# cisco/openh264

Measured on AMD Instinct MI355X. Metric: 1080p frames/sec/GPU at QP=24 CBP; encoder_binary_comparison SHA1 pass, higher is better.
Workload: dtype u8

## Files before the change

integration/welship_isvc.cpp:

```cpp
#include <dlfcn.h>
#include <stdio.h>
#include <stdlib.h>
#include <string.h>
#include <string>
#include <vector>
#include "codec_api.h"
#include "../include/welship.h"

namespace {

struct Api {
  void* so = nullptr;
  int (*Create) (WelsHipEncoder**) = nullptr;
  void (*Destroy) (WelsHipEncoder*) = nullptr;
  int (*GetDefaultParams) (WelsHipEncoder*, WelsHipEncParam*) = nullptr;
  int (*InitializeExt) (WelsHipEncoder*, const WelsHipEncParam*) = nullptr;
  int (*Uninitialize) (WelsHipEncoder*) = nullptr;
  int (*EncodeFrame) (WelsHipEncoder*, const WelsHipSourcePicture*, WelsHipFrameBSInfo*) = nullptr;
  int (*ForceIntraFrame) (WelsHipEncoder*, int) = nullptr;
  int (*GetReconFrame) (WelsHipEncoder*, uint8_t*, size_t) = nullptr;
  int (*SetOption) (WelsHipEncoder*, int, void*) = nullptr;
  int (*EncodeParameterSets) (WelsHipEncoder*, WelsHipFrameBSInfo*) = nullptr;
  int (*GetOption) (WelsHipEncoder*, int, void*) = nullptr;
  const char* (*GetLastError) (void) = nullptr;
  int (*GetFrameQuality) (WelsHipEncoder*, WelsHipFrameQuality*) = nullptr;
  bool load() {
    if (so) return true;
    const char* path = getenv ("WELSHIP_LIB");
    so = dlopen (path && *path ? path : "libwelship.so", RTLD_NOW | RTLD_LOCAL);
    if (!so) { fprintf (stderr, "welship_isvc: cannot open the engine library (%s): %s\n", path ? path : "libwelship.so", dlerror()); return false; }
#define SYM(field, name) field = reinterpret_cast<decltype (field)> (dlsym (so, name)); if (!field) { fprintf (stderr, "welship_isvc: missing symbol %s\n", name); return false; }
    SYM (Create, "WelsHipCreateEncoder") SYM (Destroy, "WelsHipDestroyEncoder") SYM (GetDefaultParams, "WelsHipGetDefaultParams")
    SYM (InitializeExt, "WelsHipInitializeExt") SYM (Uninitialize, "WelsHipUninitialize") SYM (EncodeFrame, "WelsHipEncodeFrame")
    SYM (ForceIntraFrame, "WelsHipForceIntraFrame") SYM (GetLastError, "WelsHipGetLastError") SYM (GetReconFrame, "WelsHipGetReconFrame")
    SYM (SetOption, "WelsHipSetOption") SYM (GetOption, "WelsHipGetOption") SYM (EncodeParameterSets, "WelsHipEncodeParameterSets")
    SYM (GetFrameQuality, "WelsHipGetFrameQuality")
#undef SYM
    return true;
  }
} g_api;

class CWelsHipEncoder : public ISVCEncoder {
 public:
  CWelsHipEncoder() { if (g_api.load()) g_api.Create (&m_p); }
  virtual ~CWelsHipEncoder() { if (m_p) g_api.Destroy (m_p); }
  bool Ok() const { return m_p != NULL; }

  virtual int EXTAPI Initialize (const SEncParamBase* b) {
    if (!b) return cmInitParaError;
    SEncParamExt e;
    GetDefaultParams (&e);
    e.iUsageType = b->iUsageType; e.iPicWidth = b->iPicWidth; e.iPicHeight = b->iPicHeight;
    e.iTargetBitrate = b->iTargetBitrate; e.iRCMode = b->iRCMode; e.fMaxFrameRate = b->fMaxFrameRate;
    e.sSpatialLayers[0].iVideoWidth = b->iPicWidth; e.sSpatialLayers[0].iVideoHeight = b->iPicHeight;
    e.sSpatialLayers[0].fFrameRate = b->fMaxFrameRate; e.sSpatialLayers[0].iSpatialBitrate = b->iTargetBitrate;
    return InitializeExt (&e);
  }
  virtual int EXTAPI InitializeExt (const SEncParamExt* p) {
    if (!p || !m_p) return cmInitParaError;
    WelsHipEncParam q;
    g_api.GetDefaultParams (m_p, &q);
    q.iUsageType = p->iUsageType; q.iPicWidth = p->iPicWidth; q.iPicHeight = p->iPicHeight;
    q.iTargetBitrate = p->sSpatialLayers[0].iSpatialBitrate > 0 ? p->sSpatialLayers[0].iSpatialBitrate : p->iTargetBitrate;
    q.iRCMode = p->iRCMode; q.fMaxFrameRate = p->fMaxFrameRate;
    q.iTemporalLayerNum = p->iTemporalLayerNum; q.iSpatialLayerNum = p->iSpatialLayerNum;
    q.iComplexityMode = p->iComplexityMode; q.uiIntraPeriod = p->uiIntraPeriod;
    q.eSpsPpsIdStrategy = p->eSpsPpsIdStrategy; q.iEntropyCodingModeFlag = p->iEntropyCodingModeFlag;
    q.iLoopFilterDisableIdc = p->iLoopFilterDisableIdc; q.iLoopFilterAlphaC0Offset = p->iLoopFilterAlphaC0Offset;
    q.iLoopFilterBetaOffset = p->iLoopFilterBetaOffset; q.bEnableFrameCroppingFlag = p->bEnableFrameCroppingFlag;
    const SSpatialLayerConfig& l = p->sSpatialLayers[0];
    q.iDLayerQp = l.iDLayerQp;
    q.uiSliceMode = l.sSliceArgument.uiSliceMode; q.uiSliceNum = l.sSliceArgument.uiSliceNum;
    for (int k = 0; k < MAX_SLICES_NUM_TMP && k < 35; ++k) q.uiSliceMbNum[k] = l.sSliceArgument.uiSliceMbNum[k];
    q.bEnableAdaptiveQuant = p->bEnableAdaptiveQuant; q.bEnableBackgroundDetection = p->bEnableBackgroundDetection;
    q.bEnableSceneChangeDetect = p->bEnableSceneChangeDetect; q.bEnableLongTermReference = p->bEnableLongTermReference;
    q.bEnableDenoise = p->bEnableDenoise; q.bEnableFrameSkip = p->bEnableFrameSkip;
    q.iMultipleThreadIdc = p->iMultipleThreadIdc;
    q.bPsnrY = p->bPsnrY; q.bPsnrU = p->bPsnrU; q.bPsnrV = p->bPsnrV;
    m_param_planes = (p->bPsnrY ? 1 : 0) | (p->bPsnrU ? 2 : 0) | (p->bPsnrV ? 4 : 0);
    const int rc = g_api.InitializeExt (m_p, &q);
    if (rc) fprintf (stderr, "welship_isvc: InitializeExt: %s\n", g_api.GetLastError());
    m_w = p->iPicWidth; m_h = p->iPicHeight; m_frames = 0;
    return rc;
  }
  virtual int EXTAPI GetDefaultParams (SEncParamExt* p) {
    if (!p) return cmInitParaError;
    memset (p, 0, sizeof (*p));
    WelsHipEncParam q;
    if (m_p) g_api.GetDefaultParams (m_p, &q); else memset (&q, 0, sizeof (q));
    p->iUsageType = (EUsageType)q.iUsageType; p->iRCMode = (RC_MODES)q.iRCMode; p->fMaxFrameRate = q.fMaxFrameRate;
    p->iTemporalLayerNum = q.iTemporalLayerNum; p->iSpatialLayerNum = q.iSpatialLayerNum;
    p->iComplexityMode = (ECOMPLEXITY_MODE)q.iComplexityMode; p->uiIntraPeriod = q.uiIntraPeriod;
    p->eSpsPpsIdStrategy = (EParameterSetStrategy)q.eSpsPpsIdStrategy; p->iEntropyCodingModeFlag = q.iEntropyCodingModeFlag;
    p->iLoopFilterDisableIdc = q.iLoopFilterDisableIdc; p->bEnableFrameCroppingFlag = q.bEnableFrameCroppingFlag != 0;
    p->iMultipleThreadIdc = 1; p->iNumRefFrame = 1; p->iMaxQp = 51; p->iMinQp = 0;
    p->sSpatialLayers[0].iDLayerQp = q.iDLayerQp; p->sSpatialLayers[0].uiProfileIdc = PRO_BASELINE;
    p->sSpatialLayers[0].sSliceArgument.uiSliceMode = SM_SINGLE_SLICE; p->sSpatialLayers[0].sSliceArgument.uiSliceNum = 1;
    return cmResultSuccess;
  }
  virtual int EXTAPI Uninitialize() { return m_p ? g_api.Uninitialize (m_p) : cmInitParaError; }
  virtual int EXTAPI EncodeFrame (const SSourcePicture* s, SFrameBSInfo* o) {
    if (!s || !o || !m_p) return cmInitParaError;
    WelsHipSourcePicture sp;
    memset (&sp, 0, sizeof (sp));
    sp.iColorFormat = s->iColorFormat;
    for (int k = 0; k < 4; ++k) { sp.iStride[k] = s->iStride[k]; sp.pData[k] = s->pData[k]; }
    sp.iPicWidth = s->iPicWidth; sp.iPicHeight = s->iPicHeight; sp.uiTimeStamp = s->uiTimeStamp;
    const int pic_planes = (s->bPsnrY ? 1 : 0) | (s->bPsnrU ? 2 : 0) | (s->bPsnrV ? 4 : 0);
    int planes = m_param_planes | pic_planes;
    if (g_api.SetOption (m_p, WELSHIP_OPTION_PSNR_PLANES, &planes)) return cmInitParaError;
    WelsHipFrameBSInfo b;
    const int rc = g_api.EncodeFrame (m_p, &sp, &b);
    if (rc) { fprintf (stderr, "welship_isvc: EncodeFrame: %s\n", g_api.GetLastError()); return rc; }
    memset (o, 0, sizeof (*o));
    o->iLayerNum = b.iLayerNum; o->eFrameType = (EVideoFrameType)b.eFrameType;
    o->iFrameSizeInBytes = b.iFrameSizeInBytes; o->uiTimeStamp = b.uiTimeStamp;
    for (int i = 0; i < b.iLayerNum; ++i) {
      o->sLayerInfo[i].uiLayerType = b.sLayerInfo[i].uiLayerType; o->sLayerInfo[i].eFrameType = (EVideoFrameType)b.sLayerInfo[i].eFrameType;
      o->sLayerInfo[i].uiTemporalId = b.sLayerInfo[i].uiTemporalId; o->sLayerInfo[i].uiSpatialId = b.sLayerInfo[i].uiSpatialId;
      o->sLayerInfo[i].uiQualityId = b.sLayerInfo[i].uiQualityId; o->sLayerInfo[i].iSubSeqId = b.sLayerInfo[i].iSubSeqId;
      o->sLayerInfo[i].iNalCount = b.sLayerInfo[i].iNalCount; o->sLayerInfo[i].pNalLengthInByte = b.sLayerInfo[i].pNalLengthInByte;
      o->sLayerInfo[i].pBsBuf = b.sLayerInfo[i].pBsBuf;
    }
    if (pic_planes) {
      WelsHipFrameQuality fq;
      if (g_api.GetFrameQuality (m_p, &fq)) return cmUnknownReason;
      for (int i = 0; i < b.iLayerNum; ++i)
        if (b.sLayerInfo[i].uiLayerType == WELSHIP_VIDEO_CODING_LAYER)
          for (int k = 0; k < 3; ++k) o->sLayerInfo[i].rPsnr[k] = ((pic_planes >> k) & 1) ? fq.rPsnr[k] : 0.0f;
    }
    if (!m_dump.empty() && b.eFrameType != WelsHipFrameTypeSkip) {
      std::vector<uint8_t> rec ((size_t)m_w * m_h * 3 / 2);
      if (g_api.GetReconFrame (m_p, rec.data(), rec.size()) == 0) {
        FILE* f = fopen (m_dump.c_str(), m_frames == 0 ? "wb" : "ab");
        if (f) { fwrite (rec.data(), 1, rec.size(), f); fclose (f); }
      }
    }
    ++m_frames;
    return cmResultSuccess;
  }
  virtual int EXTAPI EncodeParameterSets (SFrameBSInfo* o) {
    if (!o || !m_p) return cmInitParaError;
    WelsHipFrameBSInfo b;
    const int rc = g_api.EncodeParameterSets (m_p, &b);
    if (rc) return rc;
    memset (o, 0, sizeof (*o));
    o->iLayerNum = 1; o->eFrameType = videoFrameTypeInvalid; o->iFrameSizeInBytes = b.iFrameSizeInBytes;
    o->sLayerInfo[0].uiLayerType = NON_VIDEO_CODING_LAYER; o->sLayerInfo[0].eFrameType = videoFrameTypeInvalid;
    o->sLayerInfo[0].iNalCount = b.sLayerInfo[0].iNalCount; o->sLayerInfo[0].pNalLengthInByte = b.sLayerInfo[0].pNalLengthInByte;
    o->sLayerInfo[0].pBsBuf = b.sLayerInfo[0].pBsBuf;
    return cmResultSuccess;
  }
  virtual int EXTAPI ForceIntraFrame (bool bIdr, int = -1) { return m_p ? g_api.ForceIntraFrame (m_p, bIdr ? 1 : 0) : cmInitParaError; }
  virtual int EXTAPI SetOption (ENCODER_OPTION id, void* pOption) {
    if (id == ENCODER_OPTION_DUMP_FILE && pOption) {
      const SDumpLayer* d = static_cast<const SDumpLayer*> (pOption);
      if (d->iLayer != 0 || !d->pFileName) return cmInitParaError;
      m_dump = d->pFileName;
      return cmResultSuccess;
    }
    if (id == ENCODER_OPTION_TRACE_LEVEL || id == ENCODER_OPTION_TRACE_CALLBACK || id == ENCODER_OPTION_TRACE_CALLBACK_CONTEXT) return cmResultSuccess;
    return m_p ? g_api.SetOption (m_p, (int)id, pOption) : cmInitExpected;
  }
  virtual int EXTAPI GetOption (ENCODER_OPTION id, void* pOption) { return m_p ? g_api.GetOption (m_p, (int)id, pOption) : cmInitExpected; }

 private:
  WelsHipEncoder* m_p = NULL;
  std::string m_dump;
  int m_w = 0, m_h = 0, m_frames = 0;
  int m_param_planes = 0;
};

}

extern "C" int WelsCreateSVCEncoder (ISVCEncoder** ppEncoder) {
  if (!ppEncoder) return 1;
  CWelsHipEncoder* e = new CWelsHipEncoder();
  if (!e->Ok()) { delete e; *ppEncoder = NULL; return 1; }
  *ppEncoder = e;
  return 0;
}
extern "C" void WelsDestroySVCEncoder (ISVCEncoder* pEncoder) { delete static_cast<CWelsHipEncoder*> (pEncoder); }
```

openh264_amd/csrc/common/wh_types.h:

```cpp
#pragma once
#include <stdint.h>

#ifdef __cplusplus
extern "C" {
#endif

enum {
  WH_MB_I4x4   = 0,
  WH_MB_I16x16 = 1,
  WH_MB_P16x16 = 2,
  WH_MB_P16x8  = 3,
  WH_MB_P8x16  = 4,
  WH_MB_P8x8   = 5,
  WH_MB_PSKIP  = 6,
  WH_MB_NONE   = 255
};
#define WH_IS_INTRA(t) ((t) <= WH_MB_I16x16)
#define WH_IS_INTER(t) ((t) >= WH_MB_P16x16 && (t) <= WH_MB_PSKIP)
#define WH_REFTYPE_BACKGROUND 64

enum { WH_SLICE_P = 0, WH_SLICE_I = 2 };

typedef struct WhMbRecord {
  uint8_t  mb_type;
// ... 58 lines not shown
  const uint32_t* fme_start;
  const uint16_t* fme_loc;
  int32_t fme_list_size;
  int32_t scd_on;
  uint32_t* chain;
  uint32_t* fme_cost_down;
  uint32_t* chain_mb;
} WhSccJob;

#define WH_GOM_MAX 160

typedef struct WhGomRc {
  int32_t n_gom_mb;
  int32_t end_mb;
  int32_t target_bits;
  int32_t min_qp, max_qp;
  int32_t slice_qp;
  int32_t p_slice;
  int32_t pad;
  int32_t gom_sad[WH_GOM_MAX];
  int32_t calc_qp;
  int32_t frame_bits;
  int32_t gom_bits;
  int32_t gom_target;
  int32_t index;
  int32_t skip_run, last_qp;
  int32_t pad2;
} WhGomRc;

typedef struct WhPicJob {
  const uint8_t* src[3];
  uint8_t*       rec[3];
  const uint8_t* ref[3];
  WhMbRecord*    records;
  WhMbState*     mbs;
  const WhMbState* ref_mbs;
  int32_t        qp;
  int32_t        slice_type;
  const WhMbCtl* mb_ctl;
  int32_t        ref_is_p;
  int32_t        want_bits;
  const uint8_t* prev_src_y;
  uint32_t*      db_flags;
  uint32_t       db_gen;
  int32_t        dyn_first;
  uint32_t*      scene_count;
  int32_t*       sad_cost0;
  const int32_t* vaa_sad8x8;
  const int8_t*  bgd_flags;
  int32_t        mvc_shift;
  int32_t        mb_begin;
  int32_t        mb_end;
  int32_t        dyn_slice;
  uint8_t*       compact;
  uint32_t*      compact_off;
  const int16_t* il_hint;
  const WhSccJob* scc;
  const uint32_t* scc_order;
  const int32_t* scc_chain_prev;
  WhGomRc* gom_rc;
  int32_t*       sad_cost0_out;
  int32_t        dyn_redo;
  uint32_t       sse_planes;
  uint8_t*       rec_tiles[2];
  const uint8_t* ref_tiles[2];
  uint8_t*       rec_blk;
  uint64_t*      sse;
} WhPicJob;

#define WH_SRC_MB_BYTES 384
#define WH_SRC_Y_OFF(mb_w, mbx, mby, row, x) ((size_t) ((mby) * (mb_w) + (mbx)) * WH_SRC_MB_BYTES + (size_t) ((row) * 16 + (x)))
#define WH_SRC_C_OFF(mb_w, mbx, mby, pl, row, x) ((size_t) ((mby) * (mb_w) + (mbx)) * WH_SRC_MB_BYTES + (size_t) (256 + (pl) * 64 + (row) * 8 + (x)))
#define WH_TILE_BYTES 128
#define WH_TILE_Y_OFF(stride_y, x, y) ((((size_t) (((y) + 32) >> 3) * (size_t) ((stride_y) >> 4) + (size_t) (((x) + 32) >> 4)) << 7) + (size_t) ((((y) + 32) & 7) << 4))
#define WH_TILE_C_OFF(stride_c, x, y) ((((size_t) (((y) + 16) >> 3) * (size_t) ((stride_c) >> 3) + (size_t) (((x) + 16) >> 3)) << 7) + (size_t) ((((y) + 16) & 7) << 4))

#define WH_MAX_SLICES 36
#define WH_SEQ_SCC 1
#define WH_SEQ_SERIAL 2
#define WH_SEQ_CHAIN 4
#define WH_SEQ_PLAIN 32
#define WH_SEQ_NO_CTRL 64
#define WH_SEQ_DB_WHOLE 16
#define WH_SEQ_RANGED 8
#define WH_DB_WHOLE_TABLE(P) ((P).db_bands + 3 * (size_t)(P).db_num_bands + 1)
#define WH_DB_BAND_ROWS 24

typedef struct WhSeqParams {
  int32_t mb_w, mb_h;
  int32_t src_stride_y, src_stride_c;
  int32_t rec_stride_y, rec_stride_c;
  int32_t complexity;
  int32_t chroma_qp_offset;
  int32_t num_slices;
  int32_t slice_first_mb[WH_MAX_SLICES + 1];
  int32_t deblock_idc;
  int32_t alpha_offset, beta_offset;
  int32_t mv_range;
  int32_t flags;
  int32_t blk8_w, blk8_h;
  unsigned long long* prof;
  const uint32_t* mb_order;
  int32_t db_num_bands, db_max_mbs;
  const int32_t* db_bands;
  int32_t db_max_rows;
} WhSeqParams;

#ifdef __cplusplus
}
#endif
```

openh264_amd/csrc/hip/hip_backend.hip:

```cpp
#include <hip/hip_runtime.h>
#include <stdio.h>
#include <stdlib.h>
#include <string>
#include <vector>
#include <algorithm>
#include <map>
#include <unordered_map>
#include <atomic>
#include "../host/backend.h"
#include "../kernels/frame_kernels.h"
#include <mutex>
#include "../kernels/deblock_mb.h"
#include "../kernels/inter_mb.h"
#include "../kernels/expand_pic.h"
#include "../kernels/tile_pic.h"
#include "../kernels/vaa_pic.h"
#include "../kernels/bgd_pic.h"
#include "../kernels/scene_pic.h"
#include "../kernels/quality_pic.h"
#include "../common/compact.h"

namespace {

#define WH_NUM_QUEUES 32
#define WH_ERR_WORDS 4
#define WH_SEAM_SPIN_LIMIT (1u << 22)
#define WH_SPIN_LIMIT (1u << 23)

__device__ __forceinline__ bool wh_wait_done (const uint32_t* done, int idx, uint32_t* err) {
  if (idx < 0) return true;
  uint32_t spins = 0;
  while (!((__hip_atomic_load (&done[idx >> 5], __ATOMIC_RELAXED, __HIP_MEMORY_SCOPE_WORKGROUP) >> (idx & 31)) & 1u)) {
    __builtin_amdgcn_s_sleep (4);
    if (++spins > WH_SPIN_LIMIT) {
      if ((threadIdx.x & 63) == 0 && atomicAdd (err, 1u) == 0) { err[1] = blockIdx.x; err[2] = blockIdx.y; err[3] = (uint32_t)idx; }
      return false;
    }
  }
  return true;
}

__device__ __forceinline__ WhMbLds& wh_prof_holder (WhInterLds& S) { return S.m; }
__device__ __forceinline__ WhMbLds& wh_prof_holder (WhMbLds& S) { return S; }
__device__ __forceinline__ WhMbLds& wh_prof_holder (WhDbLds& S) { return * (WhMbLds*)&S; }
#if defined(WH_PROF)
template <class T> __device__ __forceinline__ uint32_t* wh_prof_lds (T& S) { return wh_prof_holder (S).prof; }
#define WH_PROF_ON 1
#else
template <class T> __device__ __forceinline__ uint32_t* wh_prof_lds (T& S) { return nullptr; }
#define WH_PROF_ON 0
#endif

__device__ __forceinline__ void wh_copy_job (WhPicJob* dst, const WhPicJob* src) {
  for (unsigned i = threadIdx.x; i < sizeof (WhPicJob) / 4; i += blockDim.x) ((uint32_t*)dst)[i] = ((const uint32_t*)src)[i];
}

#define WH_DEFINE_MB_KERNEL(NAME, LDS_T, BODY, MAX_THREADS, WHOLE_PICTURE, PROF, GOM)                                             \
__global__ __launch_bounds__ (MAX_THREADS) void NAME (WhSeqParams P, const WhPicJob* jobs, uint32_t* err) {             \
  extern __shared__ __align__ (16) uint8_t smem[];                                                                      \
  const int nw = (int)blockDim.x >> 6, lane = (int)threadIdx.x & 63;                                                    \
  const int wave = __builtin_amdgcn_readfirstlane ((int)threadIdx.x >> 6);      \
  LDS_T& S = ((LDS_T*)smem)[wave];                                                                                      \
  uint32_t* sched = (uint32_t*) (smem + (size_t)nw * sizeof (LDS_T));           \
  const int num_mb = P.mb_w * P.mb_h;                                                                                   \
  const int first = WHOLE_PICTURE ? 0 : P.slice_first_mb[blockIdx.x];                                                   \
  const int n = WHOLE_PICTURE ? num_mb : P.slice_first_mb[blockIdx.x + 1] - first;                                      \
  const uint32_t* order0 = P.mb_order + (WHOLE_PICTURE ? num_mb : first);                                               \
  for (int i = (int)threadIdx.x; i < 1 + ((n + 31) >> 5); i += (int)blockDim.x) sched[i] = 0;                          \
  if (WH_PROF_ON && PROF && P.prof && lane < 32) wh_prof_lds (S)[lane] = 0;                                                           \
  __shared__ WhPicJob Jl;                           \
  wh_copy_job (&Jl, &jobs[blockIdx.y]);                                                                                 \
  __syncthreads();                                                                                                      \
  WH_PROF_DECL (P);                                                                                                     \
  const WhPicJob& J = Jl;                                                                                               \
   \
   \
  const uint32_t* order = (GOM && J.gom_rc) ? (const uint32_t*)J.scc_order + first : order0;                                     \
  for (int guard = 0; guard <= n; ++guard) {                         \
    int t = 0;                                                                                                          \
    if (lane == 0) t = (int)atomicAdd (&sched[0], 1u);                                                                  \
    t = __builtin_amdgcn_readfirstlane (t);                                                                             \
    if (t >= n) break;                                                                                                  \
    const int xy = order[t];                                                                                            \
    if (PROF) WH_PROF_MARK (P, wh_prof_holder (S), 11);                                       \
    if (J.mb_end > 0) {                              \
      if (xy < J.mb_begin) { if (lane == 0) atomicOr (&sched[1 + ((xy - first) >> 5)], 1u << ((xy - first) & 31)); continue; } \
      if (xy >= J.mb_end) continue;                                                                                     \
    }                                                                                                                   \
    int dep_a, dep_b;                                                                                                   \
    wh_mb_deps (P.mb_w, xy, first, &dep_a, &dep_b);                                                                     \
    if (!wh_wait_done (sched + 1, dep_a < 0 ? -1 : dep_a - first, err)) break;        \
    if (!wh_wait_done (sched + 1, dep_b < 0 ? -1 : dep_b - first, err)) break;                                          \
    if (GOM && J.gom_rc) { const int dep_c = ((const WH_G int32_t*)J.scc_chain_prev)[xy]; if (!wh_wait_done (sched + 1, dep_c < first ? -1 : dep_c - first, err)) break; } \
    __builtin_amdgcn_fence (__ATOMIC_ACQUIRE, "workgroup");                                                             \
    if (PROF) WH_PROF_MARK (P, wh_prof_holder (S), 12);                                             \
    BODY (S, P, J, xy % P.mb_w, xy / P.mb_w);                                                                           \
    if (GOM && J.gom_rc) wh_gom_close_if_last (P, J, xy);     \
    if (PROF) WH_PROF_MARK (P, wh_prof_holder (S), 14);                \
// ... 248 lines not shown
#define WH_XCLAIM()                                                                                                            \
  {                                                                                                                            \
    int tt = 0;                                                                                                                \
    if (lane == 0) tt = (int)__hip_atomic_fetch_add (&sc[0], 1u, __ATOMIC_RELAXED, __HIP_MEMORY_SCOPE_AGENT);                  \
    tt = __builtin_amdgcn_readfirstlane (tt);                                                                                  \
    xy = -1;                                                                                                                   \
    if (tt < n) {                                                                                                              \
      xy = (int)order[tt];                                                                                                     \
      mby = P.mb_w > 1 ? (int)__umulhi ((uint32_t)xy, w_rcp) : xy; mbx = xy - mby * P.mb_w;                                    \
      WhPicJob Jf;                                                                                                             \
      Jf.src[0] = J.src[0]; Jf.prev_src_y = J.prev_src_y; Jf.ref_mbs = J.ref_mbs; Jf.ref_is_p = J.ref_is_p;                    \
      Jf.ref_tiles[0] = J.ref_tiles[0]; Jf.ref_tiles[1] = J.ref_tiles[1];                                                      \
      if (HOSTIN) { Jf.vaa_sad8x8 = J.vaa_sad8x8; Jf.sad_cost0 = J.sad_cost0; }                                                \
      const int guess_ = slot_mv;                                                                                              \
      wh_inter_cold_fetch<VAR> (S, G, lane, P, Jf, mbx, mby);                                                                  \
      wh_win_speculate (P, Jf, X.spec, mbx, mby, guess_); X.spec_valid = 1;                                                    \
    }                                                                                                                          \
  }
  WH_XCLAIM()
  while (xy >= 0) {
    const int dep_a = (mbx > 0 && xy - 1 >= first) ? xy - 1 : -1;
    int dep_b;
    { const int tr = mbx < P.mb_w - 1 ? xy - P.mb_w + 1 : xy - P.mb_w; dep_b = tr >= first ? tr : -1; }
    if (!wh_wait_done_x (sc + 1, dep_a < 0 ? -1 : dep_a - first, err)) break;
    if (!wh_wait_done_x (sc + 1, dep_b < 0 ? -1 : dep_b - first, err)) break;
    __builtin_amdgcn_fence (__ATOMIC_ACQUIRE, "workgroup");
    WV_ASYNC_WAIT();
    wh_inter_mb_body_t<false, VAR, true> (S, G, P, J, mbx, mby, X);
    asm volatile ("s_waitcnt vmcnt(0)" ::: "memory");
    if (lane == 0) __hip_atomic_fetch_or (&sc[1 + ((xy - first) >> 5)], 1u << ((xy - first) & 31), __ATOMIC_RELAXED, __HIP_MEMORY_SCOPE_SYSTEM);
    WH_XCLAIM()
  }
#undef WH_XCLAIM
#if WH_PROF_ON
  if (P.prof && lane < 32) atomicAdd (&P.prof[((blockIdx.x * 7u) & 63u) * 32u + lane], (unsigned long long)S.m.prof[lane]);
#endif
}

__global__ __launch_bounds__ (1024) void k_md_assign (uint32_t* slice_cost, uint16_t* groups, int n, int n_groups, int slots) {
  __shared__ uint32_t key[4096];
  __shared__ uint16_t val[4096];
  int m = 1;
  while (m < n) m <<= 1;
  for (int i = (int)threadIdx.x; i < m; i += (int)blockDim.x) { key[i] = i < n ? slice_cost[i] : 0u; val[i] = (uint16_t) (i < n ? i : 0xffff); }
  __syncthreads();
  for (int i = (int)threadIdx.x; i < n; i += (int)blockDim.x) slice_cost[i] = 0;
  for (int k = 2; k <= m; k <<= 1)
    for (int j = k >> 1; j > 0; j >>= 1) {
      for (int i = (int)threadIdx.x; i < m; i += (int)blockDim.x) {
        const int l = i ^ j;
        if (l > i) {
          const bool up = (i & k) == 0;
          const uint32_t a = key[i], b = key[l];
          const bool sw = up ? (a < b || (a == b && val[i] == 0xffff && val[l] != 0xffff)) : (a > b);
          if (sw) { key[i] = b; key[l] = a; const uint16_t t = val[i]; val[i] = val[l]; val[l] = t; }
        }
      }
      __syncthreads();
    }
  for (int g = (int)threadIdx.x; g < n_groups * slots; g += (int)blockDim.x) groups[g] = 0xffff;
  __shared__ int wtot[17];
  int carry = 0;
  const int lane = (int)threadIdx.x & 63, wave = (int)threadIdx.x >> 6, nwv = (int)blockDim.x >> 6;
  for (int base = 0; base < m; base += (int)blockDim.x) {
    const int i = base + (int)threadIdx.x;
    const bool valid = i < m && val[i] != 0xffff;
    const unsigned long long b = __ballot (valid);
    const int before = __builtin_popcountll (b & ((1ull << lane) - 1ull));
    __syncthreads();
    if (lane == 0) wtot[wave] = __builtin_popcountll (b);
    __syncthreads();
    if (threadIdx.x == 0) { int acc = 0; for (int w2 = 0; w2 < nwv; ++w2) { const int t = wtot[w2]; wtot[w2] = acc; acc += t; } wtot[16] = acc; }
    __syncthreads();
    if (valid) {
      const int p = carry + wtot[wave] + before;
      const int r = p / n_groups, c = p % n_groups;
      const int g = (r & 1) ? n_groups - 1 - c : c;
      if (r < slots) groups[g * slots + r] = val[i];
    }
    carry += wtot[16];
  }
}

__global__ __launch_bounds__ (1024) void k_deblock_slices (WhSeqParams P, const WhPicJob* jobs, uint32_t* err) {
  extern __shared__ __align__ (16) uint8_t smem[];
  const int nw = (int)blockDim.x >> 6, lane = (int)threadIdx.x & 63;
  const int wave = __builtin_amdgcn_readfirstlane ((int)threadIdx.x >> 6);
  WhDbLds& S = ((WhDbLds*)smem)[wave];
  WhDbXchg E;
  E.top = (uint32_t*) (smem + (size_t)nw * sizeof (WhDbLds));
  E.left = E.top + (size_t)P.mb_w * 24;
  E.first_row = 0;
  uint32_t* sched = E.left + (size_t)P.mb_h * 32;
  const int w = P.mb_w, num_mb = P.mb_w * P.mb_h;
  const int nb = P.db_num_bands;
  const int first = P.db_bands[blockIdx.x], last = P.db_bands[blockIdx.x + 1], n = last - first;
  const bool cross = P.deblock_idc == 0;
  const int sfirst = cross ? 0 : P.db_bands[nb + 1 + blockIdx.x], slast = cross ? num_mb : P.db_bands[2 * nb + 1 + blockIdx.x];
  const uint32_t* order = (P.flags & WH_SEQ_DB_WHOLE) ? P.mb_order + num_mb : P.mb_order + 2 * num_mb + first;
  for (int i = (int)threadIdx.x; i < 1 + ((n + 31) >> 5); i += (int)blockDim.x) sched[i] = 0;
  __shared__ WhPicJob Jl;
  wh_copy_job (&Jl, &jobs[blockIdx.y]);
  __syncthreads();
  const WhPicJob& J = Jl;
  uint32_t* flags = J.db_flags;
  const uint32_t gen = J.db_gen;
  __shared__ WhDbStage stage[16];
  WhDbStage& G = stage[wave];
#if WH_PROF_ON
  if (P.prof && lane < 32) S.prof[lane] = 0;
#endif
  WH_PROF_DECL (P);
  for (int guard = 0; guard <= n; ++guard) {
    int t = 0;
    if (lane == 0) t = (int)atomicAdd (&sched[0], 1u);
    t = __builtin_amdgcn_readfirstlane (t);
    if (t >= n) break;
    const int xy = order[t];
    WH_PROF_MARK (P, S, 0);
    wh_deblock_cold_fetch (G, lane, P, J, xy % w, xy / w);
    WH_PROF_MARK (P, S, 1);
    int dep_a, dep_b;
    wh_mb_deps (w, xy, 0, &dep_a, &dep_b);
    bool remote = false, ok = true;
    for (int k = 0; k < 2 && ok; ++k) {
      const int dep = k == 0 ? dep_a : dep_b;
      if (dep < 0) continue;
      if (dep >= first) ok = wh_wait_done (sched + 1, dep - first, err);
      else if (dep >= sfirst) {
        uint32_t spins = 0;
        while (__hip_atomic_load (&flags[dep], __ATOMIC_RELAXED, __HIP_MEMORY_SCOPE_SYSTEM) != gen) {
          __builtin_amdgcn_s_sleep (8);
          if (++spins > WH_SEAM_SPIN_LIMIT) { if (lane == 0 && atomicAdd (err, 1u) == 0) { err[1] = blockIdx.x; err[2] = blockIdx.y; err[3] = 0x80000000u | (uint32_t)dep; } ok = false; break; }
        }
        remote = true;
      }
    }
    if (!ok) break;
    __builtin_amdgcn_fence (__ATOMIC_ACQUIRE, "workgroup");
    WH_PROF_MARK (P, S, remote ? 3 : 2);
    WV_ASYNC_WAIT();
    WH_PROF_MARK (P, S, 4);
    const bool publish = xy + w + 1 >= last && last < slast;
    const bool drain = wh_deblock_mb_body (S, G, E, first, last, P, J, xy % w, xy / w, 0, 0, 0, publish);
    WH_PROF_MARK (P, S, 11);
    if (publish) {
      asm volatile ("s_waitcnt vmcnt(0)" ::: "memory");
      if (lane == 0) __hip_atomic_store (&flags[xy], gen, __ATOMIC_RELAXED, __HIP_MEMORY_SCOPE_SYSTEM);
    } else if (drain) {
      __builtin_amdgcn_fence (__ATOMIC_RELEASE, "workgroup");
    }
    WV_SYNC();
    if (lane == 0) atomicOr (&sched[1 + ((xy - first) >> 5)], 1u << ((xy - first) & 31));
    WH_PROF_MARK (P, S, 9);
  }
  WH_PROF_MARK (P, S, 10);
#if WH_PROF_ON
  if (P.prof && lane < 32) atomicAdd (&P.prof[2048u + ((blockIdx.x + blockIdx.y * 7u) & 63u) * 32u + lane], (unsigned long long)S.prof[lane]);
#endif
}


#ifndef WH_DB_ITEMS_IN_LDS
#define WH_DB_ITEMS_IN_LDS 1
#endif
#define WH_DB_ITEMS_LDS_MAX_MB 9216
__global__ __launch_bounds__ (1024) void k_deblock_pairs (WhSeqParams P, const WhPicJob* jobs, uint32_t* err) {
  extern __shared__ __align__ (16) uint8_t smem[];
  const int nw = (int)blockDim.x >> 6, lane = (int)threadIdx.x & 63;
  const int wave = __builtin_amdgcn_readfirstlane ((int)threadIdx.x >> 6);
  WhDbLds* S2 = (WhDbLds*)smem + 2 * wave;
  WhDbLds& S = S2[0];
  WhDbXchg E;
  E.top = (uint32_t*) (smem + (size_t)nw * 2 * sizeof (WhDbLds));
  E.left = E.top + (size_t)P.mb_w * 24;
  E.first_row = 0;
  uint32_t* sched = E.left + (size_t)P.mb_h * 32;
  const int w = P.mb_w, num_mb = P.mb_w * P.mb_h;
  const uint32_t* items_g = P.mb_order + 3 * (size_t)num_mb;
  const int n = (int)items_g[0];
  for (int i = (int)threadIdx.x; i < 1 + ((num_mb + 31) >> 5); i += (int)blockDim.x) sched[i] = 0;
#if WH_DB_ITEMS_IN_LDS
  uint32_t* items_l = sched + 1 + ((num_mb + 31) >> 5);
  const bool items_in_lds = num_mb <= WH_DB_ITEMS_LDS_MAX_MB;
  if (items_in_lds) for (int i = (int)threadIdx.x; i <= n; i += (int)blockDim.x) items_l[i] = items_g[i];
#else
  const bool items_in_lds = false; uint32_t* items_l = nullptr;
#endif
  __shared__ WhPicJob Jl;
  wh_copy_job (&Jl, &jobs[blockIdx.y]);
  __syncthreads();
  const WhPicJob& J = Jl;
  __shared__ WhDbStage stage[16][2];
  WhDbStage* G2 = stage[wave];
#if WH_PROF_ON
  if (P.prof && lane < 32) S.prof[lane] = 0;
#endif
  WH_PROF_DECL (P);
  int kind = 0, ax = 0, ay = 0;
#define WH_DB_CLAIM(KIND, X, Y) do {                                                                                     \
    int t_ = 0;                                                                                                           \
    if (lane == 0) t_ = (int)atomicAdd (&sched[0], 1u);                                                                   \
    t_ = __builtin_amdgcn_readfirstlane (t_);                                                                             \
    if (t_ >= n) KIND = 0;                                                                                                \
    else { const uint32_t it_ = WH_DB_ITEMS_IN_LDS && items_in_lds ? (uint32_t)__builtin_amdgcn_readfirstlane ((int)items_l[1 + t_]) : items_g[1 + t_]; KIND = (it_ & WH_DB_ITEM_PAIR) ? 2 : 1; X = WH_DB_ITEM_X (it_); Y = WH_DB_ITEM_Y (it_); } \
     \
     \
     \
  } while (0)
  WH_DB_CLAIM (kind, ax, ay);
  if (kind) { wh_deblock_cold_fetch (G2[0], lane, P, J, ax, ay); if (kind > 1) wh_deblock_cold_fetch (G2[1], lane, P, J, ax - 2, ay + 1); }
  WH_PROF_MARK (P, S, 0);
  for (int guard = 0; guard <= n && kind; ++guard) {
    const bool pair = kind > 1;
    const int xy = ay * w + ax, xb = xy + w - 2, bx = ax - 2, by = ay + 1;
    int dep_a, dep_b;
    wh_mb_deps (w, xy, 0, &dep_a, &dep_b);
    bool ok = wh_wait_done (sched + 1, dep_a, err) && wh_wait_done (sched + 1, dep_b, err);
    if (ok && pair) ok = wh_wait_done (sched + 1, xb - 1, err);
    if (!ok) break;
    __builtin_amdgcn_fence (__ATOMIC_ACQUIRE, "workgroup");
    WH_PROF_MARK (P, S, 2);
    WV_ASYNC_WAIT();
    WH_PROF_MARK (P, S, 4);
    if (pair && J.rec_blk) wh_deblock_pair_body (S2, G2, E, P, J, ax, ay, bx, by);
    else {
      bool drain = wh_deblock_mb_body (S, G2[0], E, 0, num_mb, P, J, ax, ay, 0, 0, 0, false);
      if (pair) drain |= wh_deblock_mb_body (S2[1], G2[1], E, 0, num_mb, P, J, bx, by, 0, 0, 0, false);
      if (drain) __builtin_amdgcn_fence (__ATOMIC_RELEASE, "workgroup");
    }
    WH_PROF_MARK (P, S, 11);
    WV_SYNC();
    if (lane == 0) {
      atomicOr (&sched[1 + (xy >> 5)], 1u << (xy & 31));
      if (pair) atomicOr (&sched[1 + (xb >> 5)], 1u << (xb & 31));
    }
    WH_PROF_MARK (P, S, 9);
    WH_DB_CLAIM (kind, ax, ay);
    if (kind) { wh_deblock_cold_fetch (G2[0], lane, P, J, ax, ay); if (kind > 1) wh_deblock_cold_fetch (G2[1], lane, P, J, ax - 2, ay + 1); }
    WH_PROF_MARK (P, S, 0);
  }
#undef WH_DB_CLAIM
  WH_PROF_MARK (P, S, 10);
#if WH_PROF_ON
  if (P.prof && lane < 32) atomicAdd (&P.prof[2048u + ((blockIdx.x + blockIdx.y * 7u) & 63u) * 32u + lane], (unsigned long long)S.prof[lane]);
#endif
}

#define WH_CP_MAX_MB 9216
__global__ __launch_bounds__ (1024) void k_compact (WhSeqParams P, const WhPicJob* jobs) {
  __shared__ uint16_t s_size[WH_CP_MAX_MB];
  __shared__ uint32_t s_mask[WH_CP_MAX_MB];
  __shared__ uint32_t s_part[1024];
  const WhPicJob J = jobs[blockIdx.x];
  if (!J.compact || !J.compact_off) return;
  const int num_mb = P.mb_w * P.mb_h, lane = (int)threadIdx.x & 63, wave = (int)threadIdx.x >> 6, nw = (int)blockDim.x >> 6;
  const WH_G WhMbRecord* recs = (const WH_G WhMbRecord*)J.records;
  for (int xy = wave; xy < num_mb; xy += nw) {
    const WH_G uint32_t* r = (const WH_G uint32_t*)&recs[xy];
    const uint32_t h0 = r[0];
    const int mb_type = (int) (h0 & 0xff), cbp = (int) ((h0 >> 8) & 0xff);
    uint32_t mask = 0;
    if (mb_type != WH_MB_PSKIP) {
      const WH_G uint32_t* c = r + 36;
#pragma unroll
      for (int k = 0; k < 4; ++k) {
        const int d = lane + 64 * k;
        const unsigned long long b = __ballot (d < 204 && c[d] != 0u);
#pragma unroll
        for (int g = 0; g < 8; ++g) if ((b >> (8 * g)) & 0xffull) { const int blk = 8 * k + g; mask |= 1u << (blk < 25 ? blk : 25); }
      }
      mask &= wh_compact_allowed (mb_type, cbp);
    }
    if (lane == 0) { s_mask[xy] = mask; s_size[xy] = (uint16_t)wh_compact_size (mb_type, mask); }
  }
  __syncthreads();
  const int per = (num_mb + (int)blockDim.x - 1) / (int)blockDim.x, t = (int)threadIdx.x;
  uint32_t sum = 0;
  for (int i = t * per; i < (t + 1) * per && i < num_mb; ++i) sum += s_size[i];
  s_part[t] = sum;
  __syncthreads();
  for (int d = 1; d < (int)blockDim.x; d <<= 1) {
    const uint32_t v = t >= d ? s_part[t - d] : 0u;
    __syncthreads();
    s_part[t] += v;
    __syncthreads();
  }
  uint32_t run = t ? s_part[t - 1] : 0u;
  for (int i = t * per; i < (t + 1) * per && i < num_mb; ++i) { J.compact_off[i] = run; run += s_size[i]; }
  if (t == (int)blockDim.x - 1) J.compact_off[num_mb] = s_part[t];
  __syncthreads();
  for (int xy = wave; xy < num_mb; xy += nw) {
    const WH_G uint32_t* r = (const WH_G uint32_t*)&recs[xy];
    WH_G uint32_t* o = (WH_G uint32_t*) ((WH_G uint8_t*)J.compact + J.compact_off[xy]);
    const uint32_t mask = s_mask[xy];
    const uint32_t h0 = r[0];
    if ((h0 & 0xff) == WH_MB_PSKIP) {
      if (lane < 2) o[lane] = r[lane];
      else if (lane == 2) o[2] = r[30];
      else if (lane == 3) o[3] = ((const WH_G uint8_t*)r)[WH_COMPACT_SIDE - 16];
      continue;
    }
    if (lane == 0) o[0] = mask;
    if (lane < 36) o[1 + lane] = r[lane];
    const WH_G uint32_t* c = r + 36;
    WH_G uint32_t* q = o + 37;
#pragma unroll
    for (int k = 0; k < 4; ++k) {
      const int d = lane + 64 * k;
      if (d < 204) {
        const int blk = d >> 3 < 25 ? d >> 3 : 25;
        if ((mask >> blk) & 1u) q[8 * __builtin_popcount (mask & ((1u << blk) - 1u)) + (d - 8 * blk)] = c[d];
      }
    }
  }
}

#define WH_CP_CHUNK 256
#define WH_CP_MAX_CHUNKS ((WH_CP_MAX_MB + WH_CP_CHUNK - 1) / WH_CP_CHUNK)
__device__ __forceinline__ uint32_t wh_cp_mask (const WH_G uint32_t* r, int lane, int mb_type, int cbp) {
  uint32_t mask = 0;
  if (mb_type != WH_MB_PSKIP) {
    const WH_G uint32_t* c = r + 36;
#pragma unroll
    for (int k = 0; k < 4; ++k) {
// ... 270 lines not shown
    const bool plain = WH_PLAIN_KERNEL && (Pin.flags & WH_SEQ_PLAIN) != 0, no_ctrl = WH_FRAME_KERNEL && (Pin.flags & WH_SEQ_NO_CTRL) != 0;
    WhSeqParams Pm = Pin;
    Pm.flags &= ~ (WH_SEQ_PLAIN | WH_SEQ_NO_CTRL);
    const WhSeqParams& P = Pm;
    static const int forced_waves = getenv ("WELSHIP_P_WAVES") ? atoi (getenv ("WELSHIP_P_WAVES")) : 0;
    static const int forced_slots = getenv ("WELSHIP_MD_SLOTS") ? atoi (getenv ("WELSHIP_MD_SLOTS")) : 0;
    const int use_assign = 1;
    const int total = P.num_slices * n;
    int slots = forced_slots > 0 ? std::min (forced_slots, WH_MD_MAX_SLOTS) : std::max (1, std::min (WH_MD_MAX_SLOTS, (total + cus_ - 1) / cus_));
    const int groups = (total + slots - 1) / slots;
    int max_n = 0, max_rows = 0;
    for (int s = 0; s < P.num_slices; ++s) {
      max_n = std::max (max_n, P.slice_first_mb[s + 1] - P.slice_first_mb[s]);
      max_rows = std::max (max_rows, (P.slice_first_mb[s + 1] - 1) / P.mb_w - P.slice_first_mb[s] / P.mb_w + 1);
    }
    const int sched_words = 1 + ((max_n + 31) >> 5);
    int nw = forced_waves > 0 ? forced_waves : WH_P_WAVES_DEFAULT;
    nw = std::min (nw, 16);
    int par = std::max (1, std::min (max_rows, (P.mb_w + 1) / 2)) * slots;
    if (P.flags & WH_SEQ_SERIAL) par = 2 * slots;
    if (P.flags & WH_SEQ_SCC) nw = std::min (nw, 6);
    nw = std::min (nw, par);
    auto built_for = [] (int w) { return w <= 6 ? 6 : w <= 12 ? 12 : w <= 14 ? 14 : 16; };
    const size_t fixed = WH_MD_MAX_SLOTS * (sizeof (WhPicJob) + 32) + 4 * (size_t)slots * sched_words;
    while (nw > 1 && (size_t)nw * sizeof (WhInterLds) + (size_t)built_for (nw) * (sizeof (WhInterStage) + sizeof (WhWinLds)) + fixed > (size_t)160 * 1024) --nw;
    const size_t lds = (size_t)nw * sizeof (WhInterLds) + 4 * (size_t)slots * sched_words;
    {
      static const int split_env = getenv ("WELSHIP_MD_SPLIT") ? atoi (getenv ("WELSHIP_MD_SPLIT")) : -1;
      const int variant = (WH_PLAIN_KERNEL == 2 && plain && P.flags == 0 && P.complexity == 0) ? 2 : (WH_PLAIN_KERNEL && plain && P.flags == 0) ? 1 : (WH_FRAME_KERNEL && no_ctrl && P.flags == 0) ? 3 : 0;
      int parts = split_env == 0 ? 1 : std::min (8, cus_ / std::max (1, total));
      if (split_env > 1) parts = std::min (split_env, 8);
      const int par1 = std::max (1, std::min (max_rows, (P.mb_w + 1) / 2));
      parts = std::min (parts, (par1 + 3 + 3) / 4);
      uint32_t* xs = (variant != 0 && parts >= 2 && forced_slots <= 0) ? split_sched ((size_t)total * sched_words) : nullptr;
      if (xs) {
        const int xw = std::max (2, std::min (WH_SPLIT_WAVES, (par1 + 3 + parts - 1) / parts));
        const size_t xlds = (size_t)xw * sizeof (WhInterLds);
        const int blocks = ((total + 7) / 8) * 8 * parts;
        HIP_TRY (hipMemsetAsync (xs, 0, 4 * (size_t)total * sched_words, stream_));
        auto xlaunch = [&] (auto kernel) {
          set_dynamic_lds ((const void*)kernel, xlds);
          if (trace_) { fprintf (stderr, "welship: MD launch, %d slices on %d CUs each, %d waves per CU\n", total, parts, xw); fflush (stderr); }
          hipLaunchKernelGGL (kernel, dim3 (blocks), dim3 (xw * 64), xlds, stream_, P, jobs, err_words(), xs, sched_words, parts, total);
          HIP_TRY (hipGetLastError());
          if (trace_) { HIP_TRY (hipStreamSynchronize (stream_)); fprintf (stderr, "welship: launch done\n"); fflush (stderr); }
        };
        if (variant == 2) xlaunch (k_inter_split<2>); else if (variant == 1) xlaunch (k_inter_split<1>); else xlaunch (k_inter_split<3>);
        return;
      }
    }
    uint16_t* grp = nullptr;
    uint32_t* cost = nullptr;
    if (slots > 1 && use_assign && total <= 4096 && stream_ == streams_[0]) {
      if ((size_t)total > md_cap_) {
        if (md_cost_) { free (md_cost_); free (md_groups_); }
        md_cap_ = (size_t)total;
        md_cost_ = (uint32_t*)alloc (4 * md_cap_);
        md_groups_ = (uint16_t*)alloc (2 * (md_cap_ + WH_MD_MAX_SLOTS));
        if (md_cost_) HIP_TRY (hipMemsetAsync (md_cost_, 0, 4 * md_cap_, stream_));
      }
      if (md_cost_ && md_groups_) {
        grp = md_groups_; cost = md_cost_;
        hipLaunchKernelGGL (k_md_assign, dim3 (1), dim3 (1024), 0, stream_, cost, grp, total, groups, slots);
        HIP_TRY (hipGetLastError());
      }
    }
    const WhSeqParams& Pr = P;
    auto launch = [&] (auto kernel) {
      set_dynamic_lds ((const void*)kernel, lds);
      if (trace_) { fprintf (stderr, "welship: MD launch %d groups x %d slots, %d waves, %zu B dynamic LDS\n", groups, slots, nw, lds); fflush (stderr); }
      hipLaunchKernelGGL (kernel, dim3 (groups), dim3 (nw * 64), lds, stream_, Pr, jobs, err_words(), (const uint16_t*)grp, slots, sched_words, total, cost);
      HIP_TRY (hipGetLastError());
      if (trace_) { HIP_TRY (hipStreamSynchronize (stream_)); fprintf (stderr, "welship: launch done\n"); fflush (stderr); }
    };
    if (P.flags & WH_SEQ_SCC) launch (k_inter_pool<384, true>);
#define WH_LAUNCH_POOL(VARIANT) do { if (nw <= 6) launch (k_inter_pool<384, false, VARIANT>); else if (nw <= 12) launch (k_inter_pool<768, false, VARIANT>); \
                                     else if (nw <= 14) launch (k_inter_pool<896, false, VARIANT>); else launch (k_inter_pool<1024, false, VARIANT>); } while (0)
    else if (WH_PLAIN_KERNEL == 2 && plain && P.flags == 0 && P.complexity == 0) WH_LAUNCH_POOL (WH_PLAIN_KERNEL == 2 ? 2 : 0);
    else if (WH_PLAIN_KERNEL && plain && P.flags == 0) WH_LAUNCH_POOL (WH_PLAIN_KERNEL ? 1 : 0);
    else if (WH_FRAME_KERNEL && no_ctrl && P.flags == 0) WH_LAUNCH_POOL (WH_FRAME_KERNEL ? 3 : 0);
    else WH_LAUNCH_POOL (0);
#undef WH_LAUNCH_POOL
  }
  void run_deblock (const WhSeqParams& P, const WhPicJob* jobs, int n) override {
    const int db_waves = 12;
    const char* we = getenv ("WELSHIP_DB_WHOLE");
    const bool whole = P.deblock_idc == 0 && P.db_bands && (P.flags & WH_SEQ_DB_WHOLE) == 0 && (we ? atoi (we) != 0 : 8 * n >= 3 * cus_);
    if (whole) {
      WhSeqParams W = P;
      W.flags |= WH_SEQ_DB_WHOLE; W.db_num_bands = 1; W.db_bands = WH_DB_WHOLE_TABLE (P); W.db_max_rows = P.mb_h; W.db_max_mbs = P.mb_w * P.mb_h;
      static const bool pairs = !(getenv ("WELSHIP_DB_PAIRS") && atoi (getenv ("WELSHIP_DB_PAIRS")) == 0);
      const size_t items_lds = (WH_DB_ITEMS_IN_LDS && P.mb_w * P.mb_h <= WH_DB_ITEMS_LDS_MAX_MB) ? 4 * ((size_t)P.mb_w * P.mb_h + 1) : 0;
      if (pairs) mb_pass (k_deblock_pairs, 2 * sizeof (WhDbLds), 16, false, W, jobs, n, 32 * sizeof (WhDbStage) + sizeof (WhPicJob), 4 * wh_db_xchg_words (P.mb_w, P.mb_h) + items_lds, 1);
      else mb_pass (k_deblock_slices, sizeof (WhDbLds), 16, false, W, jobs, n, 16 * sizeof (WhDbStage) + sizeof (WhPicJob), 4 * wh_db_xchg_words (P.mb_w, P.mb_h), 1);
      return;
    }
    mb_pass (k_deblock_slices, sizeof (WhDbLds), db_waves, false, P, jobs, n, 16 * sizeof (WhDbStage) + sizeof (WhPicJob), 4 * wh_db_xchg_words (P.mb_w, P.mb_h), P.db_num_bands);
  }
  void run_scene (const WhSeqParams& P, const WhPicJob* jobs, int n) override {
    hipLaunchKernelGGL (k_scene, dim3 (P.mb_w * P.mb_h, n), dim3 (64), 0, stream_, P, jobs);
    HIP_TRY (hipGetLastError());
  }
  void run_sse (const WhSeqParams& P, const WhPicJob* jobs, int n) override {
    if (P.mb_w > WH_SSE_MAX_MB_W) { note_error (hipErrorInvalidValue, "run_sse: picture wider than the per-lane sums allow", __LINE__); return; }
    hipLaunchKernelGGL (k_sse, dim3 ((P.mb_h + 3) / 4, n), dim3 (256), 0, stream_, P, jobs);
    HIP_TRY (hipGetLastError());
  }
  void run_qp_chain (const WhSeqParams& P, const WhPicJob* jobs, int n) override {
    hipLaunchKernelGGL (k_qp_chain, dim3 (P.num_slices, n), dim3 (64), 0, stream_, P, jobs);
    HIP_TRY (hipGetLastError());
  }
  void run_expand (const WhSeqParams& P, const WhPicJob* jobs, int n) override {
    const int blocks = std::max (1, std::min (64, (wh_expand_items (P) + 1023) / 1024));
    hipLaunchKernelGGL (k_expand, dim3 (blocks, n), dim3 (256), 0, stream_, P, jobs);
    HIP_TRY (hipGetLastError());
    hipLaunchKernelGGL (k_tile, dim3 ((wh_tile_items (P) + 255) / 256, n), dim3 (256), 0, stream_, P, jobs);
    HIP_TRY (hipGetLastError());
  }
  void run_src_tile (const WhSeqParams& P, const uint8_t* planar, uint8_t* tiled) override {
    if (!planar || !tiled) { note_null(); return; }
    hipLaunchKernelGGL (k_src_tile, dim3 ((wh_src_tile_items (P) + 255) / 256), dim3 (256), 0, stream_, P, planar, tiled);
    HIP_TRY (hipGetLastError());
  }
  void run_src_tile_jobs (const WhSeqParams& P, const WhPicJob* jobs, int n) override {
    if (!jobs || n <= 0) { note_null(); return; }
    hipLaunchKernelGGL (k_src_tile_jobs, dim3 ((wh_src_tile_items (P) + 255) / 256, n), dim3 (256), 0, stream_, P, jobs);
    HIP_TRY (hipGetLastError());
  }
  void upload_on (int q, void* dst, const void* src, size_t bytes) override {
    HIP_TRY (hipSetDevice (dev_));
    HIP_TRY (hipMemcpyAsync (dst, src, bytes, hipMemcpyHostToDevice, streams_[(q < 0 ? 0 : q) % WH_NUM_QUEUES]));
  }
  void download_on (int q, void* dst, const void* src, size_t bytes) override {
    HIP_TRY (hipSetDevice (dev_));
    HIP_TRY (hipMemcpyAsync (dst, src, bytes, hipMemcpyDeviceToHost, streams_[(q < 0 ? 0 : q) % WH_NUM_QUEUES]));
  }
  void err_snapshot (int q, uint32_t* dst) override { if (dst && usable()) { HIP_TRY (hipSetDevice (dev_)); q = (q < 0 ? 0 : q) % WH_NUM_QUEUES; HIP_TRY (hipMemcpyAsync (dst, err_ + WH_ERR_WORDS * q, 4 * WH_ERR_WORDS, hipMemcpyDeviceToHost, streams_[q])); } }
  void event_record_on (int q, void* ev) override { if (ev) { HIP_TRY (hipSetDevice (dev_)); HIP_TRY (hipEventRecord ((hipEvent_t)ev, streams_[(q < 0 ? 0 : q) % WH_NUM_QUEUES])); } }
  void queue_wait_event (int q, void* ev) override { if (ev) { HIP_TRY (hipSetDevice (dev_)); HIP_TRY (hipStreamWaitEvent (streams_[(q < 0 ? 0 : q) % WH_NUM_QUEUES], (hipEvent_t)ev, 0)); } }
  void event_wait (void* ev) override { if (ev) { HIP_TRY (hipSetDevice (dev_)); HIP_TRY (hipEventSynchronize ((hipEvent_t)ev)); } }
  void run_vaa (const WhSeqParams& P, const uint8_t* cur, const uint8_t* ref, int32_t* sad8x8, int32_t* sd8x8, uint8_t* mad8x8, int32_t* sum16, int32_t* sqsum16, int32_t* ssd16) override {
    if (!cur || !ref) { note_null(); return; }
    const WhVaaOut o = {sad8x8, sd8x8, mad8x8, sum16, sqsum16, ssd16};
    const int num_mb = P.mb_w * P.mb_h;
    hipLaunchKernelGGL (k_vaa, dim3 ((num_mb + 63) / 64), dim3 (64), 0, stream_, num_mb, cur, ref, o);
    HIP_TRY (hipGetLastError());
  }
  void run_vaa_skewed (const WhSeqParams& P, const uint8_t* cur, const uint8_t* ref, int stride, int width, int height, int32_t* sad8x8, int32_t* sd8x8, uint8_t* mad8x8,
                       int32_t* sum16, int32_t* sqsum16, int32_t* ssd16) override {
    if (!cur || !ref) { note_null(); return; }
    const WhVaaOut o = {sad8x8, sd8x8, mad8x8, sum16, sqsum16, ssd16};
    const int vw = width >> 4, vh = height >> 4;
    hipLaunchKernelGGL (k_vaa_skewed, dim3 ((vw * vh + 63) / 64), dim3 (64), 0, stream_, vw, vh, P.mb_w, stride, width, cur, ref, o);
    HIP_TRY (hipGetLastError());
  }
  void run_bgd (const WhSeqParams& P, const uint8_t* cur, const uint8_t* ref, const int32_t* sad8x8, const int32_t* sd8x8, const uint8_t* mad8x8, int units_w, int units_h,
                int8_t* flags) override {
    if (!cur || !ref || !sad8x8 || !sd8x8 || !mad8x8 || !flags) { note_null(); return; }
    const WhBgdIn in = {sad8x8, sd8x8, mad8x8, cur, ref, units_w, units_h, P.mb_w};
    const size_t lds = (size_t)units_w * units_h;
    set_dynamic_lds ((const void*)k_bgd, lds);
    hipLaunchKernelGGL (k_bgd, dim3 (1), dim3 (256), lds, stream_, in, flags);
    HIP_TRY (hipGetLastError());
  }
  void run_compact (const WhSeqParams& P, const WhPicJob* jobs, int n) override {
    const int num_mb = P.mb_w * P.mb_h, chunks = (num_mb + WH_CP_CHUNK - 1) / WH_CP_CHUNK;
    uint32_t* tot = 2 * n <= cus_ && chunks > 1 && chunks <= WH_CP_MAX_CHUNKS ? compact_totals (n) : nullptr;
    if (tot) {
      hipLaunchKernelGGL (k_compact_sizes, dim3 (chunks, n), dim3 (256), 0, stream_, P, jobs, tot);
      hipLaunchKernelGGL (k_compact_chunks, dim3 (chunks, n), dim3 (256), 0, stream_, P, jobs, (const uint32_t*)tot);
    } else
    hipLaunchKernelGGL (k_compact, dim3 (n), dim3 (1024), 0, stream_, P, jobs);
    HIP_TRY (hipGetLastError());
  }
  void queue_wait (int from) override {
    if (from < 0 || from >= (int)streams_.size() || streams_[from] == stream_ || !usable()) return;
    if (wait_ev_.empty()) wait_ev_.assign (16, nullptr);
    hipEvent_t& ev = wait_ev_[wait_next_++ % wait_ev_.size()];
    if (!ev) HIP_TRY (hipEventCreateWithFlags (&ev, hipEventDisableTiming));
    if (!ev) return;
// ... 115 lines not shown
```

openh264_amd/csrc/host/backend.h:

```cpp
#pragma once
#include <stddef.h>
#include <stdint.h>
#include "../common/wh_types.h"

namespace wh {

class Backend {
 public:
  virtual ~Backend() {}
  virtual const char* name() const = 0;
  virtual void* alloc (size_t bytes) = 0;
  virtual void free (void* p) = 0;
  virtual void upload (void* dst, const void* src, size_t bytes) = 0;
  virtual void download (void* dst, const void* src, size_t bytes) = 0;
  virtual void fill (void* dst, int value, size_t bytes) = 0;
  virtual void run_src_tile (const WhSeqParams& P, const uint8_t* planar, uint8_t* tiled) = 0;
  virtual void run_vaa (const WhSeqParams& P, const uint8_t* cur, const uint8_t* ref, int32_t* sad8x8, int32_t* sd8x8, uint8_t* mad8x8,
                        int32_t* sum16, int32_t* sqsum16, int32_t* ssd16) = 0;
  virtual void run_vaa_skewed (const WhSeqParams& P, const uint8_t* cur, const uint8_t* ref, int stride, int width, int height, int32_t* sad8x8, int32_t* sd8x8,
                               uint8_t* mad8x8, int32_t* sum16, int32_t* sqsum16, int32_t* ssd16) = 0;
  virtual void run_bgd (const WhSeqParams& P, const uint8_t* cur, const uint8_t* ref, const int32_t* sad8x8, const int32_t* sd8x8, const uint8_t* mad8x8,
                        int units_w, int units_h, int8_t* flags) = 0;
  virtual void pin_host (void* p, size_t bytes) { (void)p; (void)bytes; }
  virtual void unpin_host (void* p) { (void)p; }
  virtual void run_intra (const WhSeqParams& P, const WhPicJob* jobs, int n) = 0;
  virtual void run_inter (const WhSeqParams& P, const WhPicJob* jobs, int n) = 0;
  virtual void run_scene (const WhSeqParams& P, const WhPicJob* jobs, int n) = 0;
  virtual void run_qp_chain (const WhSeqParams& P, const WhPicJob* jobs, int n) = 0;
  virtual void run_deblock (const WhSeqParams& P, const WhPicJob* jobs, int n) = 0;
  virtual void run_expand (const WhSeqParams& P, const WhPicJob* jobs, int n) = 0;
  virtual void run_compact (const WhSeqParams& P, const WhPicJob* jobs, int n) = 0;
  virtual void run_sse (const WhSeqParams& P, const WhPicJob* jobs, int n);
  virtual void select_queue (int k) = 0;
  virtual void queue_wait (int from) { (void)from; }
  virtual int sync() = 0;
  virtual int sync_queue (int k) { (void)k; return sync(); }
  virtual unsigned errors_swept() const { return 0; }
  virtual int peek_queue_errors (int k, int via) { (void)k; (void)via; return 0; }
  virtual void upload_on (int q, void* dst, const void* src, size_t bytes) = 0;
  virtual void download_on (int q, void* dst, const void* src, size_t bytes) = 0;
  virtual void err_snapshot (int q, uint32_t* dst) { (void)q; if (dst) dst[0] = 0; }
  virtual void event_record_on (int q, void* ev) = 0;
  virtual void event_wait (void* ev) = 0;
  virtual void queue_wait_event (int q, void* ev) = 0;
  virtual void run_src_tile_jobs (const WhSeqParams& P, const WhPicJob* jobs, int n) = 0;
  virtual void* event_create() = 0;
  virtual void event_destroy (void* ev) = 0;
  virtual void event_record (void* ev) = 0;
  virtual float event_elapsed_ms (void* a, void* b) = 0;
};

Backend* create_hip_backend (int device, const char** err);

}
```

openh264_amd/csrc/host/encoder.cpp:

```cpp
#include "encoder_internal.h"
#include "quality.h"
using wh::align_up; using wh::rec_blocks_on; using wh::DevPicture;

namespace wh {
std::string& last_error() { static thread_local std::string e; return e; }
}

#define WH_PIPE_MAX_AHEAD 3

namespace {


struct SessionCore {
  wh::Backend* be = nullptr;
  WelsHipEncParam prm;
  WhSeqParams seq;
  int mb_w = 0, mb_h = 0, num_mb = 0;
  int ring = 1;
  std::vector<uint8_t*> d_src;
  uint8_t* d_src_planar = nullptr;
  DevPicture pic[WH_PIPE_MAX_AHEAD + 2];
  int nbuf = 2;
  int cur = 0;
  int ref_of (int c) const { return (c + nbuf - 1) % nbuf; }
// ... 538 lines not shown
        }
      }
      wh::write_slice_end (bw, st);
      if (!nal_fits (rbsp)) return fail_frame();
      nal_len.push_back (wh::append_nal (bs, 3, idr ? 5 : 1, rbsp));
      frame_pos += (long)rbsp.size();
    }
    if (out) {
      memset (out, 0, sizeof (*out));
      int li = 0;
      if (n_param_nals) {
        WelsHipLayerBSInfo& L = out->sLayerInfo[li++];
        L.uiLayerType = WELSHIP_NON_VIDEO_CODING_LAYER; L.eFrameType = WelsHipFrameTypeIDR;
        L.iNalCount = n_param_nals; L.pNalLengthInByte = nal_len.data(); L.pBsBuf = bs.data();
      }
      WelsHipLayerBSInfo& V = out->sLayerInfo[li++];
      V.uiLayerType = WELSHIP_VIDEO_CODING_LAYER; V.eFrameType = idr ? WelsHipFrameTypeIDR : WelsHipFrameTypeP;
      V.iSubSeqId = idr ? 0 : 3;
      V.iNalCount = s.num_slices; V.pNalLengthInByte = nal_len.data() + n_param_nals; V.pBsBuf = bs.data() + vcl_start;
      out->iLayerNum = li;
      out->eFrameType = idr ? WelsHipFrameTypeIDR : WelsHipFrameTypeP;
      out->iFrameSizeInBytes = (int32_t)bs.size();
      out->uiTimeStamp = ts;
    }
    return WELSHIP_OK;
  }

  int encode_parameter_sets (WelsHipFrameBSInfo* out) {
    if (prm.eSpsPpsIdStrategy == 1) {
      sps_id_in_bs = sps_counter % 32; pps_id_in_bs = pps_counter % 57;
      ++sps_counter; ++pps_counter;
    } else { sps_id_in_bs = 0; pps_id_in_bs = 0; }
    bs.clear();
    nal_len.clear();
    std::vector<uint8_t> rbsp;
    wh::SpsParams sp;
    sp.sps_id = sps_id_in_bs; sp.level_idc = level_idc; sp.constraint_set3 = level_1b;
    sp.width = prm.iPicWidth; sp.height = prm.iPicHeight; sp.mb_w = mb_w; sp.mb_h = mb_h;
    sp.num_ref_frames = 1; sp.gaps_in_frame_num = false; sp.frame_cropping = prm.bEnableFrameCroppingFlag != 0;
    wh::write_sps_rbsp (rbsp, sp);
    nal_len.push_back (wh::append_nal (bs, 3, 7, rbsp));
    wh::PpsParams pp;
    pp.pps_id = pps_id_in_bs; pp.sps_id = sps_id_in_bs;
    rbsp.clear();
    wh::write_pps_rbsp (rbsp, pp);
    nal_len.push_back (wh::append_nal (bs, 3, 8, rbsp));
    memset (out, 0, sizeof (*out));
    WelsHipLayerBSInfo& L = out->sLayerInfo[0];
    L.uiLayerType = WELSHIP_NON_VIDEO_CODING_LAYER; L.eFrameType = WelsHipFrameTypeInvalid;
    L.iNalCount = 2; L.pNalLengthInByte = nal_len.data(); L.pBsBuf = bs.data();
    out->iLayerNum = 1; out->eFrameType = WelsHipFrameTypeInvalid; out->iFrameSizeInBytes = (int32_t)bs.size();
    return WELSHIP_OK;
  }

  int copy_recon (uint8_t* dst, size_t bytes) {
    if (!have_recon || !dst) return WELSHIP_ERR_INIT_PARA;
    const int w = prm.iPicWidth, h = prm.iPicHeight;
    if (bytes < (size_t)w * h * 3 / 2) return WELSHIP_ERR_INIT_PARA;
    const WhSeqParams& s = seq;
    WhHostVec<uint8_t> tmp (rec_alloc_bytes + 128);
    const DevPicture& p = pic[ref_of (cur)];
    be->download (tmp.data(), p.base, rec_alloc_bytes + 128);
    be->sync();
    const uint8_t* y = tmp.data() + (p.plane[0] - p.base);
    const uint8_t* u = tmp.data() + (p.plane[1] - p.base);
    const uint8_t* v = tmp.data() + (p.plane[2] - p.base);
    for (int r = 0; r < h; ++r) memcpy (dst + (size_t)r * w, y + (size_t)r * s.rec_stride_y, w);
    uint8_t* du = dst + (size_t)w * h;
    uint8_t* dv = du + (size_t) (w / 2) * (h / 2);
    for (int r = 0; r < h / 2; ++r) {
      memcpy (du + (size_t)r * (w / 2), u + (size_t)r * s.rec_stride_c, w / 2);
      memcpy (dv + (size_t)r * (w / 2), v + (size_t)r * s.rec_stride_c, w / 2);
    }
    return WELSHIP_OK;
  }
};

static WhSeqParams plain_seq (const WhSeqParams& s) { WhSeqParams q = s; if (q.flags == 0) q.flags |= WH_SEQ_PLAIN; return q; }

void run_device_step (wh::Backend* be, const WhSeqParams& s, const WhPicJob* d_jobs, int n, bool idr, bool need_ref, bool qp_map = false, bool sse = false) {
  if (idr) be->run_intra (s, d_jobs, n);
  else be->run_inter (s, d_jobs, n);
  if (qp_map && s.deblock_idc != 1) be->run_qp_chain (s, d_jobs, n);
  if (s.deblock_idc != 1) be->run_deblock (s, d_jobs, n);
  if (need_ref) be->run_expand (s, d_jobs, n);
  if (sse) be->run_sse (s, d_jobs, n);
}

int reencode_after_overflow (wh::Backend* be, SessionCore& c, WhPicJob* d_job) {
  WhPicJob job;
  const int rc = c.retry_after_overflow (&job);
  if (rc) return rc;
  be->upload (d_job, &job, sizeof (job));
  const bool q = job.sse_planes != 0;
  if (q) be->fill (job.sse, 0, 3 * sizeof (uint64_t));
  run_device_step (be, c.seq, d_job, 1, c.cur_idr, c.prm.uiIntraPeriod != 1, true, q);
  be->download (c.h_records.data(), c.d_records, sizeof (WhMbRecord) * c.num_mb);
  if (q) be->download (c.h_sse_n[0], job.sse, 3 * sizeof (uint64_t));
  if (be->sync()) { set_err ("device scheduler timed out; the picture was not encoded"); return WELSHIP_ERR_UNKNOWN; }
  return WELSHIP_OK;
}

}

struct WelsHipEncoder {
  wh::Backend* be = nullptr;
  bool inited = false;
  SessionCore core;
  WhPicJob* d_job = nullptr;
  uint64_t* d_sse = nullptr;
  WhHostVec<uint64_t> h_sse;
};

struct WelsHipEncoderGroup {
  wh::Backend* be = nullptr;
  void parallel (int n_items, const std::function<void (int, int)>& fn) {
    const int T = host_threads < n_items ? host_threads : n_items;
    if (T <= 1) { fn (0, 1); return; }
    std::vector<std::thread> th;
    for (int t = 0; t < T; ++t) th.emplace_back ([&fn, t, T] { fn (t, T); });
    for (auto& x : th) x.join();
  }
  std::vector<std::unique_ptr<SessionCore>> sess;
  int queues = 1;
  int chunk_first (int q) const { return (int) ((long long)sess.size() * q / queues); }
  int chunk_of (int session) const { int q = 0; while (q + 1 < queues && chunk_first (q + 1) <= session) ++q; return q; }
  WhPicJob* d_jobs = nullptr;
  std::vector<WhPicJob> h_jobs;
  int host_threads = 1;
  bool pipelined = false;
  bool pipe_failed = false;
  int depth = 1;
  WhPicJob* d_jobs_n[WH_PIPE_MAX_AHEAD + 1] = {};
  WhPicJob* d_job_aux = nullptr;
  std::vector<WhPicJob> h_jobs_p[WH_PIPE_MAX_AHEAD + 1];
  long step_no = 0;
  int pending = 0;
  uint32_t* d_off_all[WH_PIPE_MAX_AHEAD + 1] = {};
  WhHostVec<uint32_t> h_off_all[WH_PIPE_MAX_AHEAD + 1];
  std::vector<void*> dl_ev;
  void* step_ev[WH_PIPE_MAX_AHEAD + 1] = {};
  void* up_ev[2][WH_PIPE_MAX_AHEAD + 1] = {};
  std::mutex stat_mu;
  double host_ms[2] = {0.0, 0.0};
  long host_pics[2] = {0, 0};
  double packed_bytes = 0.0;
  void note_host_time (int what, double ms, int pics) { std::lock_guard<std::mutex> l (stat_mu); host_ms[what] += ms; host_pics[what] += pics; }
  bool step_idr = true;
  bool mixed = false;
  std::vector<int> order;
  std::vector<int> chunk_p;
  uint64_t* d_sse_all[WH_PIPE_MAX_AHEAD + 1] = {};
  WhHostVec<uint64_t> h_sse_all[WH_PIPE_MAX_AHEAD + 1];
  std::vector<WelsHipFrameQuality> quality;
  bool have_quality = false;
  uint32_t sse_planes() const { return sess[0]->psnr_planes(); }
  bool alloc_sse (int b) {
    const size_t words = 3 * sess.size();
    d_sse_all[b] = (uint64_t*)be->alloc (sizeof (uint64_t) * words);
    if (!d_sse_all[b]) return false;
    h_sse_all[b].assign (words, 0);
    be->pin_host (h_sse_all[b].data(), sizeof (uint64_t) * words);
    for (size_t i = 0; i < sess.size(); ++i) { sess[i]->d_sse_n[b] = d_sse_all[b] + 3 * i; sess[i]->h_sse_n[b] = h_sse_all[b].data() + 3 * i; }
    return true;
  }
  void take_quality (bool pipelined_step) {
    quality.resize (sess.size());
    for (size_t i = 0; i < sess.size(); ++i) {
// ... 251 lines not shown
      if (!g->h_jobs_p[b].empty()) g->be->unpin_host (g->h_jobs_p[b].data());
      if (!g->h_off_all[b].empty()) g->be->unpin_host (g->h_off_all[b].data());
      if (g->d_off_all[b]) g->be->free (g->d_off_all[b]);
      if (b && g->d_jobs_n[b]) g->be->free (g->d_jobs_n[b]);
      g->be->event_destroy (g->step_ev[b]); g->be->event_destroy (g->up_ev[0][b]); g->be->event_destroy (g->up_ev[1][b]);
    }
    for (void* e : g->dl_ev) g->be->event_destroy (e);
    if (g->d_job_aux) g->be->free (g->d_job_aux);
    for (int b = 0; b <= WH_PIPE_MAX_AHEAD; ++b) {
      if (g->d_sse_all[b]) g->be->free (g->d_sse_all[b]);
      if (!g->h_sse_all[b].empty()) g->be->unpin_host (g->h_sse_all[b].data());
    }
  }
  g->be->free (g->d_jobs);
  delete g->be;
  delete g;
}

int WelsHipGroupUploadSource (WelsHipEncoderGroup* g, int session, int slot, const WelsHipSourcePicture* src) {
  if (!g || session < 0 || session >= (int)g->sess.size() || !src) return WELSHIP_ERR_INIT_PARA;
  SessionCore& c = *g->sess[session];
  if (slot < 0 || slot >= c.ring) return WELSHIP_ERR_INIT_PARA;
  if (src->iPicWidth != c.prm.iPicWidth || src->iPicHeight != c.prm.iPicHeight) return WELSHIP_ERR_INIT_PARA;
  g->be->select_queue (g->chunk_of (session));
  c.upload_source (slot, src);
  return WELSHIP_OK;
}

int WelsHipGroupBegin (WelsHipEncoderGroup* g, int slot) {
  if (!g) return WELSHIP_ERR_INIT_PARA;
  if (g->pipelined) { set_err ("pipelined group: frame steps go through WelsHipGroupEncodeFramesPipelined"); return WELSHIP_ERR_INIT_PARA; }
  if (g->pipe_failed) { set_err ("the group could not be made a pipelined one (out of memory) and is in an inconsistent state: destroy it"); return WELSHIP_ERR_INIT_PARA; }
  const int n = (int)g->sess.size();
  {
    std::vector<int> need;
    for (int i = 0; i < n; ++i) if (g->sess[i]->scene_check_needed()) need.push_back (i);
    if (!need.empty()) {
      g->be->select_queue (0);
      for (size_t k = 0; k < need.size(); ++k) {
        SessionCore& c = *g->sess[need[k]];
        c.scene_job (slot % c.ring, &g->h_jobs[k]);
        g->be->fill (c.d_scene, 0, 4);
      }
      g->be->upload (g->d_jobs, g->h_jobs.data(), sizeof (WhPicJob) * need.size());
      g->be->run_scene (g->sess[0]->seq, g->d_jobs, (int)need.size());
      for (int i : need) g->be->download (&g->sess[i]->h_scene, g->sess[i]->d_scene, 4);
      if (g->be->sync()) { set_err ("device error in the scene-change pass"); return WELSHIP_ERR_UNKNOWN; }
      for (int i : need) g->sess[i]->scene_verdict (g->sess[i]->h_scene);
    }
  }
  std::vector<WhPicJob> jobs (n);
  for (int i = 0; i < n; ++i) { const int rc = g->sess[i]->begin_frame_check(); if (rc) return rc; }
  for (int i = 0; i < n; ++i) { const int rc = g->sess[i]->begin_frame (slot % g->sess[i]->ring, &jobs[i]); if (rc) return rc; }
  g->step_idr = g->sess[0]->cur_idr;
  g->mixed = false;
  for (int i = 1; i < n; ++i) if (g->sess[i]->cur_idr != g->step_idr) g->mixed = true;
  g->order.resize (n);
  g->chunk_p.assign (g->queues, 0);
  for (int q = 0; q < g->queues; ++q) {
    const int a = g->chunk_first (q), b = g->chunk_first (q + 1);
    int k = a;
    for (int i = a; i < b; ++i) if (!g->sess[i]->cur_idr) g->order[k++] = i;
    g->chunk_p[q] = k - a;
    for (int i = a; i < b; ++i) if (g->sess[i]->cur_idr) g->order[k++] = i;
    for (int j = a; j < b; ++j) g->h_jobs[j] = jobs[g->order[j]];
    g->be->select_queue (q);
    g->be->upload (g->d_jobs + a, g->h_jobs.data() + a, sizeof (WhPicJob) * (b - a));
    if (g->sse_planes()) g->be->fill (g->d_sse_all[0] + 3 * (size_t)a, 0, sizeof (uint64_t) * 3 * (size_t) (b - a));
  }
  return WELSHIP_OK;
}

int WelsHipGroupRunDevice (WelsHipEncoderGroup* g, int wait) {
  if (!g) return WELSHIP_ERR_INIT_PARA;
  SessionCore& c0 = *g->sess[0];
  for (int q = 0; q < g->queues; ++q) {
    const int a = g->chunk_first (q), b = g->chunk_first (q + 1);
    g->be->select_queue (q);
    const int np = g->chunk_p[q], ni = (b - a) - np;
    const WhSeqParams& s = c0.seq;
    if (np) g->be->run_inter (plain_seq (s), g->d_jobs + a, np);
    if (ni) g->be->run_intra (s, g->d_jobs + a + np, ni);
    if (c0.use_compact) g->be->run_compact (s, g->d_jobs + a, b - a);
    if (s.deblock_idc != 1) g->be->run_deblock (s, g->d_jobs + a, b - a);
    if (c0.prm.uiIntraPeriod != 1) g->be->run_expand (s, g->d_jobs + a, b - a);
    if (g->sse_planes()) g->be->run_sse (s, g->d_jobs + a, b - a);
  }
  if (wait && g->be->sync()) { set_err ("device scheduler timed out"); return WELSHIP_ERR_UNKNOWN; }
  return WELSHIP_OK;
}

int WelsHipGroupFinish (WelsHipEncoderGroup* g, WelsHipFrameBSInfo* outs) {
  if (!g) return WELSHIP_ERR_INIT_PARA;
  const int n = (int)g->sess.size();
  const bool packed = g->sess[0]->use_compact;
  for (int i = 0; i < n; ++i) {
    SessionCore& c = *g->sess[i];
    g->be->select_queue (g->chunk_of (i));
    if (packed) g->be->download (c.h_compact_off.data(), c.d_compact_off, sizeof (uint32_t) * ((size_t)c.num_mb + 1));
    else g->be->download (c.h_records.data(), c.d_records, sizeof (WhMbRecord) * c.num_mb);
  }
  if (g->sse_planes())
    for (int q = 0; q < g->queues; ++q) {
      const size_t a = (size_t)g->chunk_first (q), b = (size_t)g->chunk_first (q + 1);
      g->be->select_queue (q);
      g->be->download (g->h_sse_all[0].data() + 3 * a, g->d_sse_all[0] + 3 * a, sizeof (uint64_t) * 3 * (b - a));
    }
  if (g->be->sync()) { set_err ("device scheduler timed out; the step was not encoded"); return WELSHIP_ERR_UNKNOWN; }
  if (packed) {
    for (int i = 0; i < n; ++i) {
      SessionCore& c = *g->sess[i];
      const size_t bytes = c.h_compact_off[c.num_mb];
      if (bytes > c.h_compact.size()) { set_err ("corrupt record offsets"); return WELSHIP_ERR_UNKNOWN; }
      g->be->select_queue (g->chunk_of (i));
      g->be->download (c.h_compact.data(), c.d_compact, bytes);
    }
    if (g->be->sync()) { set_err ("device error while copying the records"); return WELSHIP_ERR_UNKNOWN; }
  }
  for (auto& c : g->sess) c->upload_pending = false;
  std::vector<int> rcs (n, 0);
  g->parallel (n, [&] (int t, int T) {
    const auto t0 = std::chrono::steady_clock::now();
    int k = 0;
    for (int i = t; i < n; i += T, ++k) rcs[i] = g->sess[i]->finish_frame (outs ? &outs[i] : nullptr, 0, packed);
    g->note_host_time (1, std::chrono::duration<double, std::milli> (std::chrono::steady_clock::now() - t0).count(), k);
  });
  if (packed) for (auto& c : g->sess) g->packed_bytes += (double)c->h_compact_off[c->num_mb];
  for (int i = 0; i < n; ++i) {
    SessionCore& c = *g->sess[i];
    while (rcs[i] == WELSHIP_ERR_VLC_OVERFLOW) {
      g->be->select_queue (g->chunk_of (i));
      int slot = i;
      for (int k = 0; k < (int)g->order.size(); ++k) if (g->order[k] == i) { slot = k; break; }
      rcs[i] = reencode_after_overflow (g->be, c, g->d_jobs + slot);
      if (rcs[i]) break;
      rcs[i] = c.finish_frame (outs ? &outs[i] : nullptr, 0);
    }
  }
  for (int i = 0; i < n; ++i) if (rcs[i]) {
    set_err ("session " + std::to_string (i) + (rcs[i] == WELSHIP_ERR_MEMORY ? ": frame does not fit the reference encoder's bitstream buffer (cmMallocMemeError)"
                                                                             : ": entropy coding of the frame failed"));
    return rcs[i];
  }
  g->take_quality (false);
  return WELSHIP_OK;
}

int WelsHipGroupEncodeFrames (WelsHipEncoderGroup* g, const WelsHipSourcePicture* srcs, WelsHipFrameBSInfo* outs) {
  if (!g || !srcs) return WELSHIP_ERR_INIT_PARA;
  if (g->pending > 0) { set_err ("a pipelined step is pending: finish it first (WelsHipGroupEncodeFramesPipelined with no pictures)"); return WELSHIP_ERR_INIT_PARA; }
  const int n = (int)g->sess.size();
  const int slot = (g->sess[0]->last_slot + 1) % g->sess[0]->ring;
  for (int i = 0; i < n; ++i) {
    const SessionCore& c = *g->sess[i];
    if (srcs[i].iPicWidth != c.prm.iPicWidth || srcs[i].iPicHeight != c.prm.iPicHeight) return WELSHIP_ERR_INIT_PARA;
  }
  bool pending = false;
  for (int i = 0; i < n; ++i) pending = pending || g->sess[i]->upload_pending;
  if (pending) { g->be->sync(); for (auto& c : g->sess) c->upload_pending = false; }
  g->parallel (n, [&] (int t, int T) {
    const auto t0 = std::chrono::steady_clock::now();
    int k = 0;
    for (int i = t; i < n; i += T, ++k) g->sess[i]->stage_source (&srcs[i]);
    g->note_host_time (0, std::chrono::duration<double, std::milli> (std::chrono::steady_clock::now() - t0).count(), k);
  });
  for (int i = 0; i < n; ++i) { g->be->select_queue (g->chunk_of (i)); g->sess[i]->issue_upload (slot % g->sess[i]->ring); }
  int rc = WelsHipGroupBegin (g, slot);
  if (rc) return rc;
// ... 15 lines not shown
  if (g->pipelined) { if (ahead == g->depth - 1) return WELSHIP_OK; set_err ("the group is pipelined already, with a different number of steps ahead"); return WELSHIP_ERR_INIT_PARA; }
  if (g->queues != 1) { set_err ("pipelined groups use one compute queue"); return WELSHIP_ERR_UNSUPPORTED; }
  if (g->pipe_failed) { set_err ("an earlier WelsHipGroupSetPipelined failed half way: destroy the group"); return WELSHIP_ERR_INIT_PARA; }
  struct Guard { WelsHipEncoderGroup* g; bool ok = false; ~Guard() { if (!ok) g->pipe_failed = true; } } guard {g};
  const int n = (int)g->sess.size(), depth = 1 + ahead;
  const size_t off_words = (size_t)g->sess[0]->num_mb + 1;
  for (int b = 0; b < depth; ++b) {
    g->d_off_all[b] = (uint32_t*)g->be->alloc (sizeof (uint32_t) * off_words * n);
    g->h_off_all[b].assign (off_words * n, 0);
    g->be->pin_host (g->h_off_all[b].data(), sizeof (uint32_t) * off_words * n);
    g->d_jobs_n[b] = b ? (WhPicJob*)g->be->alloc (sizeof (WhPicJob) * n) : g->d_jobs;
    if (!g->d_off_all[b] || !g->d_jobs_n[b]) { set_err ("out of device memory"); return WELSHIP_ERR_MEMORY; }
    g->h_jobs_p[b].assign (n, WhPicJob());
    g->be->pin_host (g->h_jobs_p[b].data(), sizeof (WhPicJob) * n);
    g->step_ev[b] = g->be->event_create(); g->up_ev[0][b] = g->be->event_create(); g->up_ev[1][b] = g->be->event_create();
  }
  for (int i = 0; i < n; ++i) {
    uint32_t* doff[WH_PIPE_MAX_AHEAD + 1];
    uint32_t* hoff[WH_PIPE_MAX_AHEAD + 1];
    for (int b = 0; b < depth; ++b) { doff[b] = g->d_off_all[b] + off_words * i; hoff[b] = g->h_off_all[b].data() + off_words * i; }
    const int rc = g->sess[i]->enable_pipeline (ahead, doff, hoff);
    if (rc) return rc;
  }
  g->d_job_aux = (WhPicJob*)g->be->alloc (sizeof (WhPicJob));
  if (!g->d_job_aux) { set_err ("out of device memory"); return WELSHIP_ERR_MEMORY; }
  for (int b = 1; b < depth; ++b) if (!g->alloc_sse (b)) { set_err ("out of device memory"); return WELSHIP_ERR_MEMORY; }
  g->dl_ev.assign (n, nullptr);
  for (int i = 0; i < n; ++i) g->dl_ev[i] = g->be->event_create();
  if (g->be->sync()) { set_err ("device error while setting up the pipelined group"); return WELSHIP_ERR_UNKNOWN; }
  g->depth = depth;
  g->pipelined = true;
  guard.ok = true;
  return WELSHIP_OK;
}

namespace {
int pipe_submit (WelsHipEncoderGroup* g, const WelsHipSourcePicture* srcs, double* tm, const std::function<double()>& now) {
  wh::Backend* be = g->be;
  const int n = (int)g->sess.size();
  SessionCore& c0 = *g->sess[0];
  const int slot = (c0.last_slot + 1) % c0.ring;
  const int sb = (int) (g->step_no % g->depth);
  const int upq[2] = {WH_PIPE_UPQ, WH_PIPE_UPQ2 >= 0 ? WH_PIPE_UPQ2 : WH_PIPE_UPQ};
  for (int i = 0; i < n; ++i) if (srcs[i].iPicWidth != g->sess[i]->prm.iPicWidth || srcs[i].iPicHeight != g->sess[i]->prm.iPicHeight) return WELSHIP_ERR_INIT_PARA;
  for (int i = 0; i < n; ++i) { const int rc = g->sess[i]->begin_frame_check(); if (rc) return rc; }
  if (g->step_no >= g->depth) { be->event_wait (g->up_ev[0][sb]); if (upq[1] != upq[0]) be->event_wait (g->up_ev[1][sb]); }
  tm[0] = now();
  g->parallel (n, [&] (int t, int T) {
    const auto t0 = std::chrono::steady_clock::now();
    int k = 0;
    for (int i = t; i < n; i += T, ++k) g->sess[i]->stage_and_upload (&srcs[i], sb, upq[i & 1]);
    g->note_host_time (0, std::chrono::duration<double, std::milli> (std::chrono::steady_clock::now() - t0).count(), k);
  });
  be->event_record_on (upq[0], g->up_ev[0][sb]);
  if (upq[1] != upq[0]) be->event_record_on (upq[1], g->up_ev[1][sb]);
  tm[1] = now();
  std::vector<WhPicJob> jobs (n);
  for (int i = 0; i < n; ++i) {
    SessionCore& c = *g->sess[i];
    if (slot % c.ring == c.last_slot) c.prev_src_dirty = true;
    const int rc = c.begin_frame (slot % c.ring, &jobs[i]);
    if (rc) return rc;
    jobs[i].src[1] = c.planar (sb);
  }
  g->order.resize (n);
  int k = 0;
  for (int i = 0; i < n; ++i) if (!g->sess[i]->cur_idr) g->order[k++] = i;
  const int np = k;
  for (int i = 0; i < n; ++i) if (g->sess[i]->cur_idr) g->order[k++] = i;
  std::vector<WhPicJob>& hj = g->h_jobs_p[sb];
  for (int j = 0; j < n; ++j) hj[j] = jobs[g->order[j]];
  WhPicJob* dj = g->d_jobs_n[sb];
  be->select_queue (0);
  be->queue_wait_event (0, g->up_ev[0][sb]);
  if (upq[1] != upq[0]) be->queue_wait_event (0, g->up_ev[1][sb]);
  be->upload (dj, hj.data(), sizeof (WhPicJob) * n);
  const bool sse = g->sse_planes() != 0;
  if (sse) be->fill (g->d_sse_all[sb], 0, sizeof (uint64_t) * 3 * (size_t)n);
  const WhSeqParams& s = c0.seq;
  be->run_src_tile_jobs (s, dj, n);
  if (np) be->run_inter (plain_seq (s), dj, np);
  if (n - np) be->run_intra (s, dj + np, n - np);
  be->run_compact (s, dj, n);
  if (s.deblock_idc != 1) be->run_deblock (s, dj, n);
  if (c0.prm.uiIntraPeriod != 1) be->run_expand (s, dj, n);
  if (sse) be->run_sse (s, dj, n);
  be->event_record (g->step_ev[sb]);
  for (auto& c : g->sess) c->submit_advance();
  ++g->step_no;
  tm[2] = now();
  return WELSHIP_OK;
}

int pipe_finish (WelsHipEncoderGroup* g, WelsHipFrameBSInfo* outs, std::vector<int>& rcs, double* tm, const std::function<double()>& now) {
  wh::Backend* be = g->be;
  const int n = (int)g->sess.size();
  const int fb = g->sess[0]->fin.buf;
  const size_t off_words = (size_t)g->sess[0]->num_mb + 1;
  be->queue_wait_event (WH_PIPE_DLQ, g->step_ev[fb]);
  be->download_on (WH_PIPE_DLQ, g->h_off_all[fb].data(), g->d_off_all[fb], sizeof (uint32_t) * off_words * n);
  if (g->sess[0]->fin.job.sse_planes) be->download_on (WH_PIPE_DLQ, g->h_sse_all[fb].data(), g->d_sse_all[fb], sizeof (uint64_t) * 3 * (size_t)n);
  if (be->sync_queue (WH_PIPE_DLQ) || be->peek_queue_errors (0, WH_PIPE_DLQ)) { set_err ("device scheduler timed out; the step was not encoded"); return WELSHIP_ERR_UNKNOWN; }
  tm[3] = now();
  for (int i = 0; i < n; ++i) {
    SessionCore& c = *g->sess[i];
    const size_t bytes = c.hcompact_off (fb)[c.num_mb];
    if (bytes > c.hcompact (fb).size()) { set_err ("corrupt record offsets"); return WELSHIP_ERR_UNKNOWN; }
    be->download_on (WH_PIPE_DLQ, c.hcompact (fb).data(), c.dcompact (fb), bytes);
    be->event_record_on (WH_PIPE_DLQ, g->dl_ev[i]);
    g->packed_bytes += (double)bytes;
  }
  tm[4] = now();
  g->parallel (n, [&] (int t, int T) {
    double busy = 0.0;
    int k = 0;
    for (int i = t; i < n; i += T, ++k) {
      be->event_wait (g->dl_ev[i]);
      const auto t0 = std::chrono::steady_clock::now();
      rcs[i] = g->sess[i]->finish_pending (outs ? &outs[i] : nullptr);
      busy += std::chrono::duration<double, std::milli> (std::chrono::steady_clock::now() - t0).count();
    }
    g->note_host_time (1, busy, k);
  });
  tm[5] = now();
  return WELSHIP_OK;
}

int pipe_rerun (WelsHipEncoderGroup* g, SessionCore& c, WhPicJob* job, bool idr) {
  wh::Backend* be = g->be;
  if (++c.db_gen == 0) c.db_gen = 1;
  job->db_gen = c.db_gen;
  job->src[1] = nullptr;
  be->upload (g->d_job_aux, job, sizeof (WhPicJob));
  if (idr) be->run_intra (c.seq, g->d_job_aux, 1); else be->run_inter (c.seq, g->d_job_aux, 1);
  be->run_compact (c.seq, g->d_job_aux, 1);
  if (c.seq.deblock_idc != 1) be->run_deblock (c.seq, g->d_job_aux, 1);
  if (c.prm.uiIntraPeriod != 1) be->run_expand (c.seq, g->d_job_aux, 1);
  if (job->sse_planes) { be->fill (job->sse, 0, 3 * sizeof (uint64_t)); be->run_sse (c.seq, g->d_job_aux, 1); }
  if (be->sync()) { set_err ("device scheduler timed out; the picture was not encoded"); return WELSHIP_ERR_UNKNOWN; }
  return WELSHIP_OK;
}
}

int WelsHipGroupEncodeFramesPipelined (WelsHipEncoderGroup* g, const WelsHipSourcePicture* srcs, WelsHipFrameBSInfo* outs, int* pFinished) {
  if (!g || !g->pipelined) { set_err ("not a pipelined group (WelsHipGroupSetPipelined)"); return WELSHIP_ERR_INIT_PARA; }
  if (pFinished) *pFinished = 0;
  wh::Backend* be = g->be;
  const int n = (int)g->sess.size();
  const bool finish = srcs ? g->pending >= g->depth - 1 : g->pending > 0;
  static const bool trace = getenv ("WELSHIP_PIPE_TRACE") && atoi (getenv ("WELSHIP_PIPE_TRACE")) != 0;
  const auto tc0 = std::chrono::steady_clock::now();
  const std::function<double()> now = [&] () { return std::chrono::duration<double, std::milli> (std::chrono::steady_clock::now() - tc0).count(); };
  double tm[8] = {0, 0, 0, 0, 0, 0, 0, 0};
  if (srcs) {
    for (int i = 0; i < n; ++i) if (srcs[i].iPicWidth != g->sess[i]->prm.iPicWidth || srcs[i].iPicHeight != g->sess[i]->prm.iPicHeight) { set_err ("source picture size differs from the session's"); return WELSHIP_ERR_INIT_PARA; }
    for (int i = 0; i < n; ++i) { const int rc = g->sess[i]->begin_frame_check(); if (rc) return rc; }
  }
  if (finish) for (auto& c : g->sess) { c->fin = c->pendq.front(); c->pendq.pop_front(); }
  std::vector<int> rcs (n, 0);
  int frc = WELSHIP_OK, src_rc = WELSHIP_OK;
  std::string ferr;
  std::thread fth;
  if (finish) {
    if (srcs) fth = std::thread ([&] { frc = pipe_finish (g, outs, rcs, tm, now); if (frc) ferr = wh::last_error(); });
    else frc = pipe_finish (g, outs, rcs, tm, now);
    --g->pending;
  }
  const bool submitted = srcs != nullptr && (src_rc = pipe_submit (g, srcs, tm, now)) == WELSHIP_OK;
  if (fth.joinable()) { fth.join(); if (frc) set_err (ferr); }
  if (submitted) ++g->pending;
  if (trace) fprintf (stderr, "welship pipe: submit half: staging set free %.2f, staged + H2D queued %.2f, kernels queued %.2f | finish half: that step done on the device %.2f, copies queued %.2f, entropy-coded %.2f ms\n",
                      tm[0], tm[1], tm[2], tm[3], tm[4], tm[5]);
  if (frc) return frc;
  if (finish) {
    for (int i = 0; i < n; ++i) {
      if (rcs[i] != WELSHIP_ERR_VLC_OVERFLOW) continue;
      SessionCore& c = *g->sess[i];
      if (be->sync()) { set_err ("device scheduler timed out"); return WELSHIP_ERR_UNKNOWN; }
      be->select_queue (0);
      const bool need_ref = c.prm.uiIntraPeriod != 1;
      while (rcs[i] == WELSHIP_ERR_VLC_OVERFLOW) {
        WhPicJob job;
        std::swap (c.cur_job, c.fin.job);
        rcs[i] = c.retry_after_overflow (&job);
        std::swap (c.cur_job, c.fin.job);
        if (rcs[i]) break;
        job.src[1] = nullptr;
        be->upload (g->d_job_aux, &job, sizeof (job));
        if (job.sse_planes) be->fill (job.sse, 0, 3 * sizeof (uint64_t));
        run_device_step (be, c.seq, g->d_job_aux, 1, c.fin.idr, need_ref, true, job.sse_planes != 0);
        be->download (c.h_records.data(), c.d_records, sizeof (WhMbRecord) * c.num_mb);
        if (job.sse_planes) be->download (c.h_sse_n[c.fin.buf], job.sse, 3 * sizeof (uint64_t));
        if (be->sync()) { set_err ("device scheduler timed out; the picture was not encoded"); rcs[i] = WELSHIP_ERR_UNKNOWN; break; }
        rcs[i] = c.entropy_frame (outs ? &outs[i] : nullptr, 0, false, c.fin.idr, c.fin.frame_num, nullptr, nullptr);
      }
      if (!c.h_mb_ctl.empty()) memset (c.h_mb_ctl.data(), 0, sizeof (WhMbCtl) * c.h_mb_ctl.size());
      c.qp_map_in_use = false;
      for (size_t k = 0; k < c.pendq.size() && rcs[i] == WELSHIP_OK; ++k) rcs[i] = pipe_rerun (g, c, &c.pendq[k].job, c.pendq[k].idr);
      if (!c.pendq.empty()) c.cur_job = c.pendq.back().job;
    }
    for (int i = 0; i < n; ++i) if (rcs[i]) {
      set_err ("session " + std::to_string (i) + (rcs[i] == WELSHIP_ERR_MEMORY ? ": frame does not fit the reference encoder's bitstream buffer (cmMallocMemeError)"
                                                                               : ": entropy coding of the frame failed"));
      return rcs[i];
    }
    g->take_quality (true);
    if (pFinished) *pFinished = 1;
  }
  if (srcs && src_rc) return src_rc;
  return WELSHIP_OK;
}

int WelsHipGroupGetReconFrame (WelsHipEncoderGroup* g, int session, uint8_t* dst, size_t bytes) {
  if (!g || session < 0 || session >= (int)g->sess.size()) return WELSHIP_ERR_INIT_PARA;
  return g->sess[session]->copy_recon (dst, bytes);
}

const char* WelsHipGroupBackendName (WelsHipEncoderGroup* g) { return g ? g->be->name() : "none"; }

int WelsHipGroupGetFrameQuality (WelsHipEncoderGroup* g, WelsHipFrameQuality* q) {
  if (!g || !q || !g->have_quality) return WELSHIP_ERR_INIT_PARA;
  for (size_t i = 0; i < g->quality.size(); ++i) q[i] = g->quality[i];
  return WELSHIP_OK;
}

int WelsHipGroupStepDeviceOnly (WelsHipEncoderGroup* g, int slot) {
  int rc = WelsHipGroupBegin (g, slot);
  if (rc) return rc;
  WelsHipGroupRunDevice (g, 0);
  for (auto& s : g->sess) {
    s->pic[s->cur].is_p = !s->cur_idr; s->have_recon = true;
    ++s->frame_index; s->frame_num = (s->frame_num + 1) & 0x7fff; s->cur = s->next_of (s->cur);
  }
  return WELSHIP_OK;
}

int WelsHipGroupBench (WelsHipEncoderGroup* g, int steps, int warmup, double* out_ms) {
  if (!g || steps < 1 || !out_ms) return WELSHIP_ERR_INIT_PARA;
  wh::Backend* be = g->be;
  const int ring = g->sess[0]->ring;
  const int n = (int)g->sess.size();
  auto slot_of = [&] (int i) { if (ring == 1) return 0; const int period = 2 * (ring - 1); const int k = i % period; return k < ring ? k : period - k; };
  int fi = 0;
  for (int i = 0; i < warmup; ++i) { int rc = WelsHipGroupStepDeviceOnly (g, slot_of (fi++)); if (rc) return rc; }
  if (be->sync()) { set_err ("device scheduler timed out during warm-up"); return WELSHIP_ERR_UNKNOWN; }
  std::vector<void*> ev ((size_t)steps * 4 + 1);
  for (auto& e : ev) e = be->event_create();
  const WhSeqParams& s = g->sess[0]->seq;
  const bool need_ref = g->sess[0]->prm.uiIntraPeriod != 1;
  auto drop_events = [&] { for (auto& e : ev) be->event_destroy (e); };
  for (int i = 0; i < steps; ++i) {
    int rc = WelsHipGroupBegin (g, slot_of (fi++));
    if (rc) { be->sync(); drop_events(); return rc; }
    if (g->mixed) { be->sync(); drop_events(); set_err ("the benchmark entry point needs every session on the same frame type"); return WELSHIP_ERR_UNKNOWN; }
    for (int q = g->queues - 1; q >= 0; --q) {
      const int a = g->chunk_first (q), cnt = g->chunk_first (q + 1) - a;
      be->select_queue (q);
      if (q == 0) be->event_record (ev[i * 4 + 0]);
      if (g->step_idr) be->run_intra (s, g->d_jobs + a, cnt); else be->run_inter (plain_seq (s), g->d_jobs + a, cnt);
      if (q == 0) be->event_record (ev[i * 4 + 1]);
      if (s.deblock_idc != 1) be->run_deblock (s, g->d_jobs + a, cnt);
      if (q == 0) be->event_record (ev[i * 4 + 2]);
      if (need_ref) be->run_expand (s, g->d_jobs + a, cnt);
      if (q == 0) be->event_record (ev[i * 4 + 3]);
      if (g->sse_planes()) be->run_sse (s, g->d_jobs + a, cnt);
    }
    for (auto& c : g->sess) { c->pic[c->cur].is_p = !c->cur_idr; c->have_recon = true; ++c->frame_index; c->frame_num = (c->frame_num + 1) & 0x7fff; c->cur = c->next_of (c->cur); }
  }
  be->select_queue (0);
  be->event_record (ev[(size_t)steps * 4]);
  const int timed_out = be->sync();
  out_ms[0] = be->event_elapsed_ms (ev[0], ev[(size_t)steps * 4]);
  out_ms[1] = out_ms[2] = out_ms[3] = 0.0;
  for (int i = 0; i < steps; ++i) {
    out_ms[1] += be->event_elapsed_ms (ev[i * 4 + 0], ev[i * 4 + 1]);
    out_ms[2] += be->event_elapsed_ms (ev[i * 4 + 1], ev[i * 4 + 2]);
    out_ms[3] += be->event_elapsed_ms (ev[i * 4 + 2], ev[i * 4 + 3]);
  }
  drop_events();
  if (timed_out) { set_err ("device scheduler timed out during the benchmark; the timings are invalid"); return WELSHIP_ERR_UNKNOWN; }
  return WELSHIP_OK;
}

int WelsHipGroupHostStats (WelsHipEncoderGroup* g, double* out4) {
  if (!g || !out4) return WELSHIP_ERR_INIT_PARA;
  std::lock_guard<std::mutex> l (g->stat_mu);
  out4[0] = g->host_pics[0] ? g->host_ms[0] / (double)g->host_pics[0] : 0.0;
  out4[1] = g->host_pics[1] ? g->host_ms[1] / (double)g->host_pics[1] : 0.0;
  out4[2] = (double)g->host_pics[1];
  out4[3] = g->host_pics[1] ? g->packed_bytes / (double)g->host_pics[1] : 0.0;
  return WELSHIP_OK;
}

int WelsHipGroupProfile (WelsHipEncoderGroup* g, int enable, unsigned long long* out64) {
  if (!g) return WELSHIP_ERR_INIT_PARA;
  wh::Backend* be = g->be;
  unsigned long long*& prof = g->sess[0]->seq.prof;
  const size_t bytes = 2 * 64 * 32 * 8 + 64 + 256 * 8;
  if (enable && !prof) { prof = (unsigned long long*)be->alloc (bytes); be->fill (prof, 0, bytes); be->sync(); }
  if (out64 && prof) {
    std::vector<unsigned long long> h (2 * 64 * 32 + 8 + 256);
    be->download (h.data(), prof, bytes); be->sync(); be->fill (prof, 0, bytes); be->sync();
    for (int k = 0; k < 2; ++k)
      for (int i = 0; i < 32; ++i) { out64[k * 32 + i] = 0; for (int b = 0; b < 64; ++b) out64[k * 32 + i] += h[(size_t)k * 2048 + (size_t)b * 32 + i]; }
    out64[44] = h[4097] ? h[4097] - ~h[4096] : 0; out64[45] = h[4098]; out64[46] = h[4099];
  }
  if (!enable && prof) { be->free (prof); prof = nullptr; }
  return WELSHIP_OK;
}

}
```

openh264_amd/csrc/host/frame_api.cpp:

```cpp
#include "encoder_internal.h"
using wh::align_up; using wh::rec_blocks_on; using wh::DevPicture;

namespace {

struct FrameLayout {
  int mb_w = 0, mb_h = 0, idc = -1;
  std::vector<int32_t> slices;
  uint32_t* d_order = nullptr;
  int32_t* d_bands = nullptr;
  int nb = 0, max_mbs = 0, max_rows = 0;
};

struct FrameItem;
struct FrameLane {
  int queue = 0;
  bool busy = false;
  WhPicJob* d_jobs = nullptr;
  int jobs_cap = 0;
  std::vector<WhPicJob> h_jobs;
  void* tail_ev = nullptr;
  std::vector<uint32_t> h_err;
  void* tail_done_ev[2] = {nullptr, nullptr};
  std::vector<uint32_t> h_err_tail;
  unsigned tail_slot = 0;
// ... 220 lines not shown
    for (int i = 0; i < WH_MAX_SLICES + 1; ++i) s.slice_first_mb[i] = i <= n ? first[i] : 0;
    s.mb_order = L->d_order;
    s.db_num_bands = L->nb; s.db_bands = L->d_bands; s.db_max_mbs = L->max_mbs; s.db_max_rows = L->max_rows;
    return WELSHIP_OK;
  }
};

namespace {

struct FrameItem {
  WelsHipFrameCtx* c = nullptr;
  bool packed = false;
  WhSeqParams seq;
  WhPicJob job;
  bool is_p = false, qp_map = false, expand = false;
  int cur_pic = 0;
  int32_t* sad_dst = nullptr;
  bool done = false;
  int rc = 0;
};

void FrameLane::fail_tails() {
  for (WelsHipFrameCtx* x : tail_ctxs) { x->tail_failed = true; x->tail_lane = nullptr; }
  tail_ctxs.clear();
}

void frame_run_batch (FrameShared* sh, FrameKey* K, FrameLane* L, std::unique_lock<std::mutex>& lock, std::vector<FrameItem*>& batch) {
  wh::Backend* be = sh->be;
  const auto t_launch0 = std::chrono::steady_clock::now();
  const int n = (int)batch.size();
  be->select_queue (L->queue);
  be->queue_wait (K->queue);
  for (FrameItem* x : batch) x->c->join_tail (L->queue);
  if (n > L->jobs_cap) {
    if (L->d_jobs) be->free (L->d_jobs);
    if (!L->h_jobs.empty()) be->unpin_host (L->h_jobs.data());
    L->jobs_cap = std::max (16, 2 * n);
    L->d_jobs = (WhPicJob*)be->alloc (sizeof (WhPicJob) * L->jobs_cap);
    L->h_jobs.assign (L->jobs_cap, WhPicJob());
    be->pin_host (L->h_jobs.data(), sizeof (WhPicJob) * L->jobs_cap);
  }
  int rc_all = L->d_jobs ? WELSHIP_OK : WELSHIP_ERR_MEMORY;
  if (rc_all == WELSHIP_OK) {
    bool any_packed = false;
    for (int i = 0; i < n; ++i) {
      L->h_jobs[i] = batch[i]->job;
      L->h_jobs[i].compact = batch[i]->packed ? batch[i]->c->d_compact : nullptr;
      L->h_jobs[i].compact_off = batch[i]->packed ? batch[i]->c->d_compact_off : nullptr;
      any_packed = any_packed || batch[i]->packed;
    }
    be->upload (L->d_jobs, L->h_jobs.data(), sizeof (WhPicJob) * n);
    const WhSeqParams& s = K->seq;
    if (K->is_p) {
      bool no_ctrl = s.flags == 0;
      for (int i = 0; i < n && no_ctrl; ++i) {
        const WhPicJob& q = L->h_jobs[i];
        no_ctrl = !q.il_hint && !q.mb_ctl && !q.gom_rc && !q.dyn_slice && !q.want_bits && !q.mb_end && !q.scc;
      }
      WhSeqParams sq = s;
      if (no_ctrl) sq.flags |= WH_SEQ_NO_CTRL;
      be->run_inter (sq, L->d_jobs, n);
    } else be->run_intra (s, L->d_jobs, n);
    if (K->qp_map) be->run_qp_chain (s, L->d_jobs, n);
    if (any_packed) be->run_compact (s, L->d_jobs, n);
    for (FrameItem* x : batch) {
      WelsHipFrameCtx* c = x->c;
      if (x->packed) {
        c->compact_got = std::min (c->compact_est, c->h_compact.size());
        be->download (c->h_coff.data(), c->d_compact_off, sizeof (uint32_t) * (c->num_mb + 1));
        be->download (c->h_compact.data(), c->d_compact, c->compact_got);
      } else
      be->download (c->h_records.data(), c->d_records, sizeof (WhMbRecord) * c->num_mb);
      if (x->sad_dst) be->download (c->h_sad_out.data(), x->job.sad_cost0_out ? x->job.sad_cost0_out : x->job.sad_cost0, sizeof (int32_t) * c->num_mb);
      if (c->scc_active) be->download (c->scc_down(), c->d_scc_chain + 4 * WH_MAX_SLICES, sizeof (uint32_t) * WH_MAX_SLICES);
    }
    const int q = L->queue;
    static const bool tail_env_off = getenv ("WELSHIP_FRAME_TAIL") && atoi (getenv ("WELSHIP_FRAME_TAIL")) == 0;
    const bool tail = !tail_env_off && (s.deblock_idc != 1 || K->expand);
    if (tail) {
      if (!L->tail_ev) { L->tail_ev = be->event_create(); L->h_err.assign (4, 0u); be->pin_host (L->h_err.data(), 16); }
      be->err_snapshot (q, L->h_err.data());
      be->event_record_on (q, L->tail_ev);
    }
    if (s.deblock_idc != 1) be->run_deblock (s, L->d_jobs, n);
    if (K->expand) be->run_expand (s, L->d_jobs, n);
    for (FrameItem* x : batch) x->c->tail_queue = tail && L->tail_ev ? q : -1;
    if (tail && L->tail_ev) {
      if (L->h_err_tail.empty()) { L->h_err_tail.assign (8, 0u); be->pin_host (L->h_err_tail.data(), 32); for (void*& e : L->tail_done_ev) e = be->event_create(); }
      const int slot = (int) (++L->tail_slot & 1);
      be->err_snapshot (q, L->h_err_tail.data() + 4 * slot);
      be->event_record_on (q, L->tail_done_ev[slot]);
      for (FrameItem* x : batch) {
        WelsHipFrameCtx* c = x->c;
        if (c->tail_lane && c->tail_lane != L) c->tail_lane->tail_ctxs.erase (std::remove (c->tail_lane->tail_ctxs.begin(), c->tail_lane->tail_ctxs.end(), c), c->tail_lane->tail_ctxs.end());
        if (c->tail_lane != L) L->tail_ctxs.push_back (c);
        c->tail_lane = L; c->tail_slot = slot;
      }
    }
    const double launch_ms = std::chrono::duration<double, std::milli> (std::chrono::steady_clock::now() - t_launch0).count();
    const unsigned swept0 = be->errors_swept();
    lock.unlock();
    const auto t_dev0 = std::chrono::steady_clock::now();
    int bad = 0;
    if (tail && L->tail_ev) {
      be->event_wait (L->tail_ev);
      bad = L->h_err[0] != 0;
      if (bad) (void)be->sync_queue (q);
    } else bad = be->sync_queue (q);
    if (be->errors_swept() != swept0) bad = 1;
    const double dev_ms = std::chrono::duration<double, std::milli> (std::chrono::steady_clock::now() - t_dev0).count();
    lock.lock();
    if (!bad && any_packed) {
      bool more = false;
      for (FrameItem* x : batch) if (x->packed) {
        WelsHipFrameCtx* c = x->c;
        const size_t total = c->h_coff[c->num_mb];
        if (total > c->h_compact.size()) { bad = 1; continue; }
        if (total > c->compact_got) {
          if (!more) { be->select_queue (q); more = true; }
          be->download (c->h_compact.data() + c->compact_got, c->d_compact + c->compact_got, total - c->compact_got);
        }
        c->compact_est = std::min (c->h_compact.size(), ((total + total / 4 + 4095) & ~ (size_t)4095) + 65536);
      }
      if (more) { lock.unlock(); if (be->sync_queue (q)) bad = 1; lock.lock(); }
    }
    if (bad) {
      for (FrameItem* x : batch) { x->c->tail_lane = nullptr; L->tail_ctxs.erase (std::remove (L->tail_ctxs.begin(), L->tail_ctxs.end(), x->c), L->tail_ctxs.end()); }
      L->fail_tails();
    }
    if ((int)sh->stat_n.size() <= n) { sh->stat_n.resize (n + 1, 0); sh->stat_dev_ms.resize (n + 1, 0.0); sh->stat_gather_ms.resize (n + 1, 0.0); sh->stat_launch_ms.resize (n + 1, 0.0); }
    ++sh->stat_n[n]; sh->stat_dev_ms[n] += dev_ms; sh->stat_launch_ms[n] += launch_ms;
    if (bad) rc_all = WELSHIP_ERR_UNKNOWN;
    ++sh->batches; sh->batched_pictures += n;
  }
  for (FrameItem* it : batch) {
    it->rc = rc_all;
    if (rc_all == WELSHIP_OK) { it->c->pics[it->cur_pic].is_p = it->is_p; it->c->h_pic_of = -1; }
    it->done = true;
  }
}

FrameKey* frame_find_key (FrameShared* sh, const WhSeqParams& s, bool is_p, bool qp_map, bool expand) {
  for (auto& k : sh->keys)
    if (k->is_p == is_p && k->qp_map == qp_map && k->expand == expand && memcmp (&k->seq, &s, sizeof (WhSeqParams)) == 0) return k.get();
  std::unique_ptr<FrameKey> k (new FrameKey());
  k->seq = s; k->is_p = is_p; k->qp_map = qp_map; k->expand = expand;
  const int kn = (int) (sh->keys.size() % 8);
  k->queue = kn;
  for (int i = 0; i < WH_FRAME_LANES; ++i) k->lane[i].queue = 8 + 8 * i + 4 * (kn / 4) + (3 - kn % 4);
  if (kn < 2 && sh->keys.size() < 2) k->lane[1].queue = 8 + 8 + (3 - kn % 4 + 3) % 4;
  sh->keys.push_back (std::move (k));
  return sh->keys.back().get();
}

}

extern "C" {

int WelsHipFrameCtxCreate (WelsHipFrameCtx** pp, const WelsHipFrameCfg* cfg) {
  if (!pp || !cfg) return WELSHIP_ERR_INIT_PARA;
  if (cfg->iPicWidth < 16 || cfg->iPicHeight < 16 || cfg->iPicWidth > 4096 || cfg->iPicHeight > 2304 || cfg->iNumPictures < 2 || cfg->iNumPictures > 64) {
    set_err ("invalid frame context configuration"); return WELSHIP_ERR_INIT_PARA;
  }
  FrameShared* sh = nullptr;
  {
    std::lock_guard<std::mutex> reg (g_frame_registry_mu);
    for (FrameShared* x : g_frame_shared) if (x->device == cfg->iDevice) sh = x;
    if (!sh) {
// ... 346 lines not shown
    if (scc_chain && !c->d_scc_order) c->d_scc_order = (uint32_t*)A (8 * (size_t)c->num_mb + 64);
    if (dyn && scc_chain && !c->d_scc_chain_mb) c->d_scc_chain_mb = (uint32_t*)A (16 * (size_t)c->num_mb + 64);
    if (scc_entries > c->scc_loc_cap) { if (c->d_scc_loc) be->free (c->d_scc_loc); c->d_scc_loc = (uint16_t*)A (4 * scc_entries + 64); c->scc_loc_cap = scc_entries; }
    if (oom) { set_err ("out of device memory"); return WELSHIP_ERR_MEMORY; }
    if (first_part) {
      const uint8_t* st = c->h_scc.data();
      be->upload (c->d_scc_idc, st, (size_t)4 * c->num_mb);
      if (scr->pRefOriChroma[0] && scr->pRefOriChroma[1]) be->upload (c->d_scc_ori, st + scc_off_ori, 2 * c->csz);
      if (scc_lists) { be->upload (c->d_scc_lists, st + scc_off_times, 8 * scc_lists); be->upload (c->d_scc_loc, st + scc_off_loc, 4 * scc_entries); }
      if (scc_chain) be->upload (c->d_scc_order, st + scc_off_order, 8 * (size_t)c->num_mb);
      be->fill (c->d_scc_chain, 0, sizeof (uint32_t) * 5 * WH_MAX_SLICES);
      WhSccJob& z = c->scc_job();
      memset (&z, 0, sizeof (z));
      z.static_idc = c->d_scc_idc;
      const bool have_ori = scr->pRefOriChroma[0] && scr->pRefOriChroma[1];
      z.ref_ori_c[0] = have_ori ? c->d_scc_ori : nullptr; z.ref_ori_c[1] = have_ori ? c->d_scc_ori + c->csz : nullptr;
      z.scroll_flag = scr->bScrollDetectFlag ? 1 : 0; z.scroll_mvx = scr->iScrollMvX; z.scroll_mvy = scr->iScrollMvY;
      z.thr16 = scr->uiSadCostThreshold16x16; z.thr8 = scr->uiSadCostThreshold8x8;
      z.fme = scc_lists ? 1 : 0;
      z.scd_on = scr->bStaticSkipDecision ? 1 : 0;
      z.fme_times = c->d_scc_lists; z.fme_start = c->d_scc_lists ? c->d_scc_lists + scc_lists : nullptr; z.fme_loc = c->d_scc_loc;
      z.fme_list_size = (int32_t)scc_lists;
      z.chain = c->d_scc_chain; z.fme_cost_down = c->d_scc_chain + 4 * WH_MAX_SLICES;
      z.chain_mb = c->d_scc_chain_mb;
      be->upload (c->d_scc, &z, sizeof (z));
    }
    if (retry) be->fill (c->d_scc_chain, 0, sizeof (uint32_t) * 5 * WH_MAX_SLICES);
  }
  DevPicture& cur = c->pics[j->iCurPic];
  WhPicJob job;
  memset (&job, 0, sizeof (job));
  job.src[0] = job.src[1] = job.src[2] = c->d_src;
  for (int i = 0; i < 3; ++i) { job.rec[i] = cur.plane[i]; job.ref[i] = is_p ? c->pics[j->iRefPic].plane[i] : nullptr; }
  for (int i = 0; i < 2; ++i) { job.rec_tiles[i] = cur.tiles[i]; job.ref_tiles[i] = is_p ? c->pics[j->iRefPic].tiles[i] : nullptr; }
  job.records = c->d_records;
  job.rec_blk = s.deblock_idc != 1 ? c->d_rec_blk : nullptr;
  job.mbs = cur.mbs;
  job.ref_mbs = is_p ? c->pics[j->iRefPic].mbs : nullptr;
  job.qp = j->iQp;
  job.slice_type = is_p ? WH_SLICE_P : WH_SLICE_I;
  job.mb_ctl = (qp_map && !gom) ? c->d_mb_ctl : nullptr;
  job.ref_is_p = is_p && c->pics[j->iRefPic].is_p ? 1 : 0;
  job.want_bits = j->bCountBits ? (1 | (is_p && j->iNumRefIdxL0Active > 1 ? 2 : 0)) : 0;
  job.prev_src_y = nullptr;
  job.db_flags = c->d_dbflags;
  job.db_gen = c->db_gen;
  job.sad_cost0 = c->d_sad_cost0;
  if (dyn) {
    if (j->pSadCost) { set_err ("size-limited slices: single-layer sessions only"); return WELSHIP_ERR_INIT_PARA; }
    if (!c->d_sad_cost0_new) { c->d_sad_cost0_new = (int32_t*)be->alloc (sizeof (int32_t) * c->num_mb); if (c->d_sad_cost0_new) be->fill (c->d_sad_cost0_new, 0, sizeof (int32_t) * c->num_mb); }
    if (!c->d_sad_cost0_new) { set_err ("out of device memory"); return WELSHIP_ERR_MEMORY; }
    job.sad_cost0_out = c->d_sad_cost0_new;
    job.dyn_redo = j->bDynRedoFirst ? 1 : 0;
  } else if (!ranged) {
    if (!c->d_sad_cost0_new) { c->d_sad_cost0_new = (int32_t*)be->alloc (sizeof (int32_t) * c->num_mb); if (c->d_sad_cost0_new) be->fill (c->d_sad_cost0_new, 0, sizeof (int32_t) * c->num_mb); }
    if (!c->d_sad_cost0_new) { set_err ("out of device memory"); return WELSHIP_ERR_MEMORY; }
    job.sad_cost0_out = c->d_sad_cost0_new;
    c->sad_swap_pending = true;
  }
  job.vaa_sad8x8 = is_p && j->pVaaSad8x8 ? c->d_vaa : nullptr;
  job.bgd_flags = is_p && j->pBgdFlags ? c->d_bgd : nullptr;
  job.mvc_shift = j->iMvcShift;
  job.il_hint = is_p && j->pIlHint ? c->d_il : nullptr;
  job.scc = scr ? c->d_scc : nullptr;
  job.scc_order = scc_chain ? c->d_scc_order : nullptr;
  job.scc_chain_prev = scc_chain ? (const int32_t*) (c->d_scc_order + c->num_mb) : nullptr;
  if (gom) {
    job.gom_rc = c->d_gom_rc;
    job.scc_order = (const uint32_t*) ((const uint8_t*)c->d_gom_rc + sizeof (WhGomRc));
    job.scc_chain_prev = (const int32_t*) (job.scc_order + c->num_mb);
    job.want_bits |= 1 | (j->iNumRefIdxL0Active > 1 ? 2 : 0);
  }
  job.mb_begin = ranged ? j->iMbBegin : 0; job.mb_end = ranged ? j->iMbEnd : 0;
  job.dyn_slice = dyn ? j->iDynSlice : 0; job.dyn_first = dyn ? j->iDynSliceFirstMb : 0;

  if (ranged) {
    if (!dyn_close) {
      be->upload (c->d_job, &job, sizeof (job));
      if (is_p) be->run_inter (s, c->d_job, 1); else be->run_intra (s, c->d_job, 1);
    }
    if (last_part) {
      job.mb_begin = 0; job.mb_end = 0; be->sync_queue (queue); be->upload (c->d_job, &job, sizeof (job));
      if (qp_map) be->run_qp_chain (s, c->d_job, 1);
      if (s.deblock_idc != 1) be->run_deblock (s, c->d_job, 1);
      if (j->bExpand) be->run_expand (s, c->d_job, 1);
      cur.is_p = is_p;
      if (dyn) std::swap (c->d_sad_cost0, c->d_sad_cost0_new);
      if (j->pSadCost) be->download (j->pSadCost, c->d_sad_cost0, sizeof (int32_t) * c->num_mb);
      if (scr) be->download (c->scc_down(), c->d_scc_chain + 4 * WH_MAX_SLICES, sizeof (uint32_t) * WH_MAX_SLICES);
    }
    if (!dyn_close) be->download (c->h_records.data() + j->iMbBegin, c->d_records + j->iMbBegin, sizeof (WhMbRecord) * (size_t) (j->iMbEnd - j->iMbBegin));
    const unsigned swept0 = be->errors_swept();
    lock.unlock();
    int bad = be->sync_queue (queue);
    if (be->errors_swept() != swept0) bad = 1;
    lock.lock();
    c->tail_queue = -1;
    if (bad) { set_err ("device scheduler timed out or device error; the picture was not encoded"); return WELSHIP_ERR_UNKNOWN; }
    if (scr && last_part && scr->pSliceFMECostDown) memcpy (scr->pSliceFMECostDown, c->scc_down(), sizeof (uint32_t) * j->iNumSlices);
    *pp_records = c->h_records.data();
    return WELSHIP_OK;
  }

  FrameItem item;
  item.c = c; item.seq = s; item.job = job; item.is_p = is_p; item.qp_map = qp_map; item.expand = j->bExpand != 0;
  item.cur_pic = j->iCurPic; item.sad_dst = j->pSadCost;
  static const bool compact_off_env = getenv ("WELSHIP_COMPACT") && atoi (getenv ("WELSHIP_COMPACT")) == 0;
  if (j->bPackedRecords && c->num_mb <= WELSHIP_PACKED_MAX_MB && !compact_off_env) {
    if (!c->d_compact) {
      c->d_compact = (uint8_t*)be->alloc ((size_t)c->num_mb * WH_COMPACT_MAX_BYTES);
      c->d_compact_off = (uint32_t*)be->alloc (sizeof (uint32_t) * ((size_t)c->num_mb + 1));
      if (!c->d_compact || !c->d_compact_off) { set_err ("out of device memory"); return WELSHIP_ERR_MEMORY; }
      c->h_compact.resize ((size_t)c->num_mb * WH_COMPACT_MAX_BYTES);
      c->h_coff.resize ((size_t)c->num_mb + 1);
      be->pin_host (c->h_compact.data(), c->h_compact.size());
      be->pin_host (c->h_coff.data(), sizeof (uint32_t) * c->h_coff.size());
      c->compact_est = c->h_compact.size() / 4;
    }
    item.packed = true;
  }
  c->last_key = K;
  c->last_submit = std::chrono::steady_clock::now();
  sh->stat_submit_ms += std::chrono::duration<double, std::milli> (c->last_submit - t_sub0).count();
  K->pending.push_back (&item);
  if (K->gathering) sh->cv.notify_all();
  for (;;) {
    if (item.done) break;
    const int li = K->free_lane();
    if (li >= 0 && K->gathering == 0 && !K->pending.empty() && (K->next_leader == nullptr || K->next_leader == &item)) {
      FrameLane* Lk = &K->lane[li];
      Lk->busy = true;
      ++K->gathering;
      K->next_leader = nullptr;
      const auto t_g0 = std::chrono::steady_clock::now();
      if (sh->gather_us > 0 && sh->ctxs.size() > 1) {
        const auto now = std::chrono::steady_clock::now();
        size_t expected = 0;
        for (WelsHipFrameCtx* x : sh->ctxs) if (x->last_key == K && now - x->last_submit < std::chrono::milliseconds (100)) ++expected;
        if (K->pending.size() < expected)
          sh->cv.wait_for (lock, std::chrono::microseconds (sh->gather_us), [&] { return K->pending.size() >= expected; });
      }
      std::vector<FrameItem*> batch;
      batch.swap (K->pending);
      K->next_leader = nullptr;
      --K->gathering;
      const double gather_ms = std::chrono::duration<double, std::milli> (std::chrono::steady_clock::now() - t_g0).count();
      const size_t bn = batch.size();
      frame_run_batch (sh, K, Lk, lock, batch);
      if (bn < sh->stat_gather_ms.size()) sh->stat_gather_ms[bn] += gather_ms;
      Lk->busy = false;
      if (!K->pending.empty() && K->gathering == 0 && K->next_leader == nullptr) K->next_leader = K->pending.front();
      sh->cv.notify_all();
      continue;
    }
    sh->cv.wait (lock);
  }
  if (item.rc) { set_err ("device scheduler timed out or device error; the picture was not encoded"); return item.rc; }
  lock.unlock();
  if (j->pSadCost) memcpy (j->pSadCost, c->h_sad_out.data(), sizeof (int32_t) * c->num_mb);
  if (scr && scr->pSliceFMECostDown) memcpy (scr->pSliceFMECostDown, c->scc_down(), sizeof (uint32_t) * j->iNumSlices);
  if (item.packed) {
    c->packed_view.pData = c->h_compact.data(); c->packed_view.pOffset = c->h_coff.data();
    *pp_records = &c->packed_view;
    *j->pbRecordsPacked = 1;
  } else *pp_records = c->h_records.data();
  return WELSHIP_OK;
}

// ... 173 lines not shown
```

openh264_amd/csrc/kernels/expand_pic.h:

```cpp
#pragma once
#include "prims.h"

WH_HDFN void wh_expand_plane_geom (const WhSeqParams& P, int pl, int* w, int* h, int* pad, int* stride) {
  if (pl == 0) { *w = P.mb_w * 16; *h = P.mb_h * 16; *pad = 32; *stride = P.rec_stride_y; }
  else { *w = P.mb_w * 8; *h = P.mb_h * 8; *pad = 16; *stride = P.rec_stride_c; }
}
WH_HDFN int wh_expand_plane_items (int w, int h, int pad) { return h * (pad >> 1) + 2 * pad * ((w + 2 * pad) >> 2); }
WH_HDFN int wh_expand_items (const WhSeqParams& P) {
  return wh_expand_plane_items (P.mb_w * 16, P.mb_h * 16, 32) + 2 * wh_expand_plane_items (P.mb_w * 8, P.mb_h * 8, 16);
}

WH_HDFN void wh_expand_item (const WhSeqParams& P, WH_G uint8_t* rec0, WH_G uint8_t* rec1, WH_G uint8_t* rec2, int idx) {
  int pl = 0, w, h, pad, stride;
  wh_expand_plane_geom (P, 0, &w, &h, &pad, &stride);
  const int n0 = wh_expand_plane_items (w, h, pad);
  if (idx >= n0) {
    idx -= n0;
    wh_expand_plane_geom (P, 1, &w, &h, &pad, &stride);
    const int n1 = wh_expand_plane_items (w, h, pad);
    pl = 1;
    if (idx >= n1) { idx -= n1; pl = 2; }
  }
  WH_G uint8_t* base = pl == 0 ? rec0 : pl == 1 ? rec1 : rec2;
  const int side_items = h * (pad >> 1), per_side = pad >> 2;
  if (idx < side_items) {
    const int r = idx / (2 * per_side), k = idx - r * 2 * per_side, right = k >= per_side, j = k - right * per_side;
    const uint32_t v = 0x01010101u * base[(ptrdiff_t)r * stride + (right ? w - 1 : 0)];
    * (WH_G uint32_t*) (base + (ptrdiff_t)r * stride + (right ? w + 4 * j : -pad + 4 * j)) = v;
    return;
  }
  idx -= side_items;
  const int per_row = (w + 2 * pad) >> 2;
  const int r = idx / per_row, x = -pad + 4 * (idx - r * per_row);
  const bool top = r < pad;
  const WH_G uint8_t* srow = base + (ptrdiff_t) (top ? 0 : h - 1) * stride;
  const uint32_t v = x < 0 ? 0x01010101u * srow[0] : x >= w ? 0x01010101u * srow[w - 1] : * (const WH_G uint32_t*) (srow + x);
  * (WH_G uint32_t*) (base + (ptrdiff_t) (top ? r - pad : h + r - pad) * stride + x) = v;
}
```

openh264_amd/csrc/kernels/tile_pic.h:

```cpp
#pragma once
#include "prims.h"

WH_HDFN int wh_tile_items_y (const WhSeqParams& P) { return (P.rec_stride_y >> 4) * ((P.mb_h * 16 + 64) >> 3) * 8; }
WH_HDFN int wh_tile_items_c (const WhSeqParams& P) { return (P.rec_stride_c >> 3) * ((P.mb_h * 8 + 32) >> 3) * 8; }
WH_HDFN int wh_tile_items (const WhSeqParams& P) { return wh_tile_items_y (P) + wh_tile_items_c (P); }

WH_HDFN void wh_tile_copy_y (const WhSeqParams& P, const WhPicJob& J, int tx, int ty, int row) {
  const int tw = P.rec_stride_y >> 4;
  const WH_G uint8_t* src = (const WH_G uint8_t*)J.rec[0] - (ptrdiff_t)32 * P.rec_stride_y - 32 + (ptrdiff_t) (ty * 8 + row) * P.rec_stride_y + tx * 16;
  wh_stg16 ((WH_G uint8_t*)J.rec_tiles[0] + ((size_t) (ty * tw + tx) * 8 + row) * 16, wh_ldg16 (src));
}
WH_HDFN void wh_tile_copy_c (const WhSeqParams& P, const WhPicJob& J, int tx, int ty, int row) {
  const int tw = P.rec_stride_c >> 3;
  const ptrdiff_t off = - (ptrdiff_t)16 * P.rec_stride_c - 16 + (ptrdiff_t) (ty * 8 + row) * P.rec_stride_c + tx * 8;
  const WH_G uint32_t* cb = (const WH_G uint32_t*) ((const WH_G uint8_t*)J.rec[1] + off);
  const WH_G uint32_t* cr = (const WH_G uint32_t*) ((const WH_G uint8_t*)J.rec[2] + off);
  WhU4 v;
  v.x = cb[0]; v.y = cb[1]; v.z = cr[0]; v.w = cr[1];
  wh_stg16 ((WH_G uint8_t*)J.rec_tiles[1] + ((size_t) (ty * tw + tx) * 8 + row) * 16, v);
}
WH_HDFN void wh_tile_item (const WhSeqParams& P, const WhPicJob& J, int idx) {
  const int ny = wh_tile_items_y (P);
  if (idx < ny) { const int tw = P.rec_stride_y >> 4, tile = idx >> 3; wh_tile_copy_y (P, J, tile % tw, tile / tw, idx & 7); return; }
  idx -= ny;
  const int tw = P.rec_stride_c >> 3, tile = idx >> 3;
  wh_tile_copy_c (P, J, tile % tw, tile / tw, idx & 7);
}
WH_HDFN int wh_tile_border_tiles (int tw, int th, int in_w, int in_h) { return tw * (th - in_h) + in_h * (tw - in_w); }
WH_HDFN int wh_tile_border_items_y (const WhSeqParams& P) { return 8 * wh_tile_border_tiles (P.rec_stride_y >> 4, (P.mb_h * 16 + 64) >> 3, P.mb_w, 2 * P.mb_h); }
WH_HDFN int wh_tile_border_items_c (const WhSeqParams& P) { return 8 * wh_tile_border_tiles (P.rec_stride_c >> 3, (P.mb_h * 8 + 32) >> 3, P.mb_w, P.mb_h); }
WH_HDFN int wh_tile_border_items (const WhSeqParams& P) { return wh_tile_border_items_y (P) + wh_tile_border_items_c (P); }
WH_HDFN void wh_tile_border_tile (int t, int tw, int th, int top, int in_w, int in_h, int* tx, int* ty) {
  const int above = top * tw, below = (th - top - in_h) * tw;
  if (t < above) { *ty = t / tw; *tx = t - *ty * tw; return; }
  t -= above;
  if (t < below) { const int r = t / tw; *ty = top + in_h + r; *tx = t - r * tw; return; }
  t -= below;
  const int side = tw - in_w, r = t / side, c = t - r * side;
  *ty = top + r; *tx = c < 2 ? c : c + in_w;
}
WH_HDFN void wh_tile_border_item (const WhSeqParams& P, const WhPicJob& J, int idx) {
  const int ny = wh_tile_border_items_y (P);
  int tx, ty;
  if (idx < ny) { wh_tile_border_tile (idx >> 3, P.rec_stride_y >> 4, (P.mb_h * 16 + 64) >> 3, 4, P.mb_w, 2 * P.mb_h, &tx, &ty); wh_tile_copy_y (P, J, tx, ty, idx & 7); return; }
  idx -= ny;
  wh_tile_border_tile (idx >> 3, P.rec_stride_c >> 3, (P.mb_h * 8 + 32) >> 3, 2, P.mb_w, P.mb_h, &tx, &ty);
  wh_tile_copy_c (P, J, tx, ty, idx & 7);
}

WH_HDFN int wh_src_tile_items (const WhSeqParams& P) { return P.mb_w * P.mb_h * 24; }
WH_HDFN void wh_src_tile_item (const WhSeqParams& P, const WH_G uint8_t* planar, WH_G uint8_t* tiled, int idx) {
  const int xy = idx / 24, i = idx - xy * 24, mbx = xy % P.mb_w, mby = xy / P.mb_w;
  const size_t ysz = (size_t)P.src_stride_y * P.mb_h * 16, csz = (size_t)P.src_stride_c * P.mb_h * 8;
  WhU4 v;
  if (i < 16) v = wh_ldg16 (planar + (size_t) (mby * 16 + i) * P.src_stride_y + mbx * 16);
  else {
    const int pl = (i - 16) >> 2, r = ((i - 16) & 3) * 2;
    const WH_G uint32_t* a = (const WH_G uint32_t*) (planar + ysz + pl * csz + (size_t) (mby * 8 + r) * P.src_stride_c + mbx * 8);
    const WH_G uint32_t* b = (const WH_G uint32_t*) ((const WH_G uint8_t*)a + P.src_stride_c);
    v.x = a[0]; v.y = a[1]; v.z = b[0]; v.w = b[1];
  }
  wh_stg16 (tiled + (size_t)idx * 16, v);
}
```

Measured before the change: 27790.

## Fuse reference border expansion and border tiling into the deblocking kernel

Adds a fused path where deblocking workgroups, once their macroblock work drains, pull border chunks from an atomic queue. Each chunk waits on per-edge-MB written bits tracked in LDS, then pads the picture borders and updates the border tiles. This removes the separate expand kernel launch and its pass over the reconstructed picture. In exchange it adds LDS bitmaps, atomics and spin-waits on deblock completion, and the tail of the deblock kernel may be lengthened.

```diff
diff --git a/integration/welship_isvc.cpp b/integration/welship_isvc.cpp
--- a/integration/welship_isvc.cpp
+++ b/integration/welship_isvc.cpp
@@ -106,7 +106,9 @@
     sp.iColorFormat = s->iColorFormat;
     for (int k = 0; k < 4; ++k) { sp.iStride[k] = s->iStride[k]; sp.pData[k] = s->pData[k]; }
     sp.iPicWidth = s->iPicWidth; sp.iPicHeight = s->iPicHeight; sp.uiTimeStamp = s->uiTimeStamp;
-    const int pic_planes = (s->bPsnrY ? 1 : 0) | (s->bPsnrU ? 2 : 0) | (s->bPsnrV ? 4 : 0);
+    unsigned char fy, fu, fv;
+    memcpy (&fy, &s->bPsnrY, 1); memcpy (&fu, &s->bPsnrU, 1); memcpy (&fv, &s->bPsnrV, 1);
+    const int pic_planes = (fy != 0 ? 1 : 0) | (fu != 0 ? 2 : 0) | (fv != 0 ? 4 : 0);
     int planes = m_param_planes | pic_planes;
     if (g_api.SetOption (m_p, WELSHIP_OPTION_PSNR_PLANES, &planes)) return cmInitParaError;
     WelsHipFrameBSInfo b;
diff --git a/openh264_amd/csrc/common/wh_types.h b/openh264_amd/csrc/common/wh_types.h
--- a/openh264_amd/csrc/common/wh_types.h
+++ b/openh264_amd/csrc/common/wh_types.h
@@ -164,6 +164,7 @@
 #define WH_SEQ_PLAIN 32
 #define WH_SEQ_NO_CTRL 64
 #define WH_SEQ_DB_WHOLE 16
+#define WH_SEQ_DB_EXPAND 128
 #define WH_SEQ_RANGED 8
 #define WH_DB_WHOLE_TABLE(P) ((P).db_bands + 3 * (size_t)(P).db_num_bands + 1)
 #define WH_DB_BAND_ROWS 24
diff --git a/openh264_amd/csrc/hip/hip_backend.hip b/openh264_amd/csrc/hip/hip_backend.hip
--- a/openh264_amd/csrc/hip/hip_backend.hip
+++ b/openh264_amd/csrc/hip/hip_backend.hip
@@ -14,6 +14,7 @@
 #include "../kernels/inter_mb.h"
 #include "../kernels/expand_pic.h"
 #include "../kernels/tile_pic.h"
+#include "../kernels/border_pic.h"
 #include "../kernels/vaa_pic.h"
 #include "../kernels/bgd_pic.h"
 #include "../kernels/scene_pic.h"
@@ -428,6 +429,31 @@
   }
 }
 
+__device__ __forceinline__ bool wh_db_is_edge_mb (const WhSeqParams& P, int mbx, int mby) { return mbx == 0 || mby == 0 || mbx == P.mb_w - 1 || mby == P.mb_h - 1; }
+__device__ __forceinline__ void wh_db_set_written (uint32_t* written, int xy, int lane) {
+  if (lane == 0) atomicOr (&written[xy >> 5], 1u << (xy & 31));
+}
+__device__ __forceinline__ void wh_db_border_chunks (const WhSeqParams& P, const WhPicJob& J, uint32_t* border, uint32_t* err, int lane) {
+  const int total = wh_border_chunks (P);
+  for (int guard = 0; guard <= total; ++guard) {
+    int c = 0;
+    if (lane == 0) c = (int)atomicAdd (&border[0], 1u);
+    c = __builtin_amdgcn_readfirstlane (c);
+    if (c >= total) break;
+    const WhBorderChunk C = wh_border_chunk (P, c);
+    bool ok = true;
+#pragma unroll
+    for (int i = 0; i < WH_BORDER_MAX_DEPS; ++i) if (ok) ok = wh_wait_done (border + 1, C.deps[i], err);
+    if (!ok) break;
+    __builtin_amdgcn_fence (__ATOMIC_ACQUIRE, "workgroup");
+    wh_border_chunk_expand (P, J, C, lane, 64);
+    __builtin_amdgcn_fence (__ATOMIC_RELEASE, "workgroup");
+    asm volatile ("s_waitcnt vmcnt(0)" ::: "memory");
+    __builtin_amdgcn_fence (__ATOMIC_ACQUIRE, "workgroup");
+    wh_border_chunk_tiles (P, J, C, lane, 64);
+  }
+}
+
 __global__ __launch_bounds__ (1024) void k_deblock_slices (WhSeqParams P, const WhPicJob* jobs, uint32_t* err) {
   extern __shared__ __align__ (16) uint8_t smem[];
   const int nw = (int)blockDim.x >> 6, lane = (int)threadIdx.x & 63;
@@ -439,12 +465,16 @@
   E.first_row = 0;
   uint32_t* sched = E.left + (size_t)P.mb_h * 32;
   const int w = P.mb_w, num_mb = P.mb_w * P.mb_h;
+  const bool fuse = (P.flags & WH_SEQ_DB_EXPAND) != 0;
+  uint32_t* border = sched + 1 + ((num_mb + 31) >> 5);
+  int pend = -1;
   const int nb = P.db_num_bands;
   const int first = P.db_bands[blockIdx.x], last = P.db_bands[blockIdx.x + 1], n = last - first;
   const bool cross = P.deblock_idc == 0;
   const int sfirst = cross ? 0 : P.db_bands[nb + 1 + blockIdx.x], slast = cross ? num_mb : P.db_bands[2 * nb + 1 + blockIdx.x];
   const uint32_t* order = (P.flags & WH_SEQ_DB_WHOLE) ? P.mb_order + num_mb : P.mb_order + 2 * num_mb + first;
   for (int i = (int)threadIdx.x; i < 1 + ((n + 31) >> 5); i += (int)blockDim.x) sched[i] = 0;
+  if (fuse) for (int i = (int)threadIdx.x; i < 1 + ((num_mb + 31) >> 5); i += (int)blockDim.x) border[i] = 0;
   __shared__ WhPicJob Jl;
   wh_copy_job (&Jl, &jobs[blockIdx.y]);
   __syncthreads();
@@ -486,6 +516,7 @@
     __builtin_amdgcn_fence (__ATOMIC_ACQUIRE, "workgroup");
     WH_PROF_MARK (P, S, remote ? 3 : 2);
     WV_ASYNC_WAIT();
+    if (fuse && pend >= 0) { wh_db_set_written (border + 1, pend, lane); pend = -1; }
     WH_PROF_MARK (P, S, 4);
     const bool publish = xy + w + 1 >= last && last < slast;
     const bool drain = wh_deblock_mb_body (S, G, E, first, last, P, J, xy % w, xy / w, 0, 0, 0, publish);
@@ -498,7 +529,14 @@
     }
     WV_SYNC();
     if (lane == 0) atomicOr (&sched[1 + ((xy - first) >> 5)], 1u << ((xy - first) & 31));
+    if (fuse && wh_db_is_edge_mb (P, xy % w, xy / w)) pend = xy;
     WH_PROF_MARK (P, S, 9);
+  }
+  if (fuse) {
+    __builtin_amdgcn_fence (__ATOMIC_RELEASE, "workgroup");
+    asm volatile ("s_waitcnt vmcnt(0)" ::: "memory");
+    if (pend >= 0) wh_db_set_written (border + 1, pend, lane);
+    wh_db_border_chunks (P, J, border, err, lane);
   }
   WH_PROF_MARK (P, S, 10);
 #if WH_PROF_ON
@@ -525,9 +563,12 @@
   const int w = P.mb_w, num_mb = P.mb_w * P.mb_h;
   const uint32_t* items_g = P.mb_order + 3 * (size_t)num_mb;
   const int n = (int)items_g[0];
-  for (int i = (int)threadIdx.x; i < 1 + ((num_mb + 31) >> 5); i += (int)blockDim.x) sched[i] = 0;
+  const bool fuse = (P.flags & WH_SEQ_DB_EXPAND) != 0;
+  uint32_t* border = sched + 1 + ((num_mb + 31) >> 5);
+  int pend = -1;
+  for (int i = (int)threadIdx.x; i < 2 * (1 + ((num_mb + 31) >> 5)); i += (int)blockDim.x) sched[i] = 0;
 #if WH_DB_ITEMS_IN_LDS
-  uint32_t* items_l = sched + 1 + ((num_mb + 31) >> 5);
+  uint32_t* items_l = border + 1 + ((num_mb + 31) >> 5);
   const bool items_in_lds = num_mb <= WH_DB_ITEMS_LDS_MAX_MB;
   if (items_in_lds) for (int i = (int)threadIdx.x; i <= n; i += (int)blockDim.x) items_l[i] = items_g[i];
 #else
@@ -568,6 +609,7 @@
     __builtin_amdgcn_fence (__ATOMIC_ACQUIRE, "workgroup");
     WH_PROF_MARK (P, S, 2);
     WV_ASYNC_WAIT();
+    if (fuse && pend >= 0) { wh_db_set_written (border + 1, pend, lane); pend = -1; }
     WH_PROF_MARK (P, S, 4);
     if (pair && J.rec_blk) wh_deblock_pair_body (S2, G2, E, P, J, ax, ay, bx, by);
     else {
@@ -581,12 +623,19 @@
       atomicOr (&sched[1 + (xy >> 5)], 1u << (xy & 31));
       if (pair) atomicOr (&sched[1 + (xb >> 5)], 1u << (xb & 31));
     }
+    if (fuse && !pair && wh_db_is_edge_mb (P, ax, ay)) pend = xy;
     WH_PROF_MARK (P, S, 9);
     WH_DB_CLAIM (kind, ax, ay);
     if (kind) { wh_deblock_cold_fetch (G2[0], lane, P, J, ax, ay); if (kind > 1) wh_deblock_cold_fetch (G2[1], lane, P, J, ax - 2, ay + 1); }
     WH_PROF_MARK (P, S, 0);
   }
 #undef WH_DB_CLAIM
+  if (fuse) {
+    __builtin_amdgcn_fence (__ATOMIC_RELEASE, "workgroup");
+    asm volatile ("s_waitcnt vmcnt(0)" ::: "memory");
+    if (pend >= 0) wh_db_set_written (border + 1, pend, lane);
+    wh_db_border_chunks (P, J, border, err, lane);
+  }
   WH_PROF_MARK (P, S, 10);
 #if WH_PROF_ON
   if (P.prof && lane < 32) atomicAdd (&P.prof[2048u + ((blockIdx.x + blockIdx.y * 7u) & 63u) * 32u + lane], (unsigned long long)S.prof[lane]);
@@ -1023,7 +1072,14 @@
     else WH_LAUNCH_POOL (0);
 #undef WH_LAUNCH_POOL
   }
-  void run_deblock (const WhSeqParams& P, const WhPicJob* jobs, int n) override {
+  void run_deblock (const WhSeqParams& P, const WhPicJob* jobs, int n) override { (void)deblock (P, jobs, n, false); }
+  bool run_deblock_expand (const WhSeqParams& P, const WhPicJob* jobs, int n) override { return deblock (P, jobs, n, true); }
+  bool deblock (const WhSeqParams& Pin, const WhPicJob* jobs, int n, bool expand) {
+#if defined(WH_AB_SWITCHES)
+    if (expand && getenv ("WELSHIP_FUSE_BORDER") && atoi (getenv ("WELSHIP_FUSE_BORDER")) == 0) expand = false;
+#endif
+    WhSeqParams P = Pin;
+    const size_t border_lds = 4 * (size_t) (1 + ((P.mb_w * P.mb_h + 31) >> 5));
     const int db_waves = 12;
     const char* we = getenv ("WELSHIP_DB_WHOLE");
     const bool whole = P.deblock_idc == 0 && P.db_bands && (P.flags & WH_SEQ_DB_WHOLE) == 0 && (we ? atoi (we) != 0 : 8 * n >= 3 * cus_);
@@ -1032,11 +1088,15 @@
       W.flags |= WH_SEQ_DB_WHOLE; W.db_num_bands = 1; W.db_bands = WH_DB_WHOLE_TABLE (P); W.db_max_rows = P.mb_h; W.db_max_mbs = P.mb_w * P.mb_h;
       static const bool pairs = !(getenv ("WELSHIP_DB_PAIRS") && atoi (getenv ("WELSHIP_DB_PAIRS")) == 0);
       const size_t items_lds = (WH_DB_ITEMS_IN_LDS && P.mb_w * P.mb_h <= WH_DB_ITEMS_LDS_MAX_MB) ? 4 * ((size_t)P.mb_w * P.mb_h + 1) : 0;
-      if (pairs) mb_pass (k_deblock_pairs, 2 * sizeof (WhDbLds), 16, false, W, jobs, n, 32 * sizeof (WhDbStage) + sizeof (WhPicJob), 4 * wh_db_xchg_words (P.mb_w, P.mb_h) + items_lds, 1);
-      else mb_pass (k_deblock_slices, sizeof (WhDbLds), 16, false, W, jobs, n, 16 * sizeof (WhDbStage) + sizeof (WhPicJob), 4 * wh_db_xchg_words (P.mb_w, P.mb_h), 1);
-      return;
-    }
-    mb_pass (k_deblock_slices, sizeof (WhDbLds), db_waves, false, P, jobs, n, 16 * sizeof (WhDbStage) + sizeof (WhPicJob), 4 * wh_db_xchg_words (P.mb_w, P.mb_h), P.db_num_bands);
+      if (expand) W.flags |= WH_SEQ_DB_EXPAND;
+      if (pairs) mb_pass (k_deblock_pairs, 2 * sizeof (WhDbLds), 16, false, W, jobs, n, 32 * sizeof (WhDbStage) + sizeof (WhPicJob), 4 * wh_db_xchg_words (P.mb_w, P.mb_h) + items_lds + border_lds, 1);
+      else mb_pass (k_deblock_slices, sizeof (WhDbLds), 16, false, W, jobs, n, 16 * sizeof (WhDbStage) + sizeof (WhPicJob), 4 * wh_db_xchg_words (P.mb_w, P.mb_h) + (expand ? border_lds : 0), 1);
+      return expand;
+    }
+    if (P.db_num_bands != 1) expand = false;
+    if (expand) P.flags |= WH_SEQ_DB_EXPAND;
+    mb_pass (k_deblock_slices, sizeof (WhDbLds), db_waves, false, P, jobs, n, 16 * sizeof (WhDbStage) + sizeof (WhPicJob), 4 * wh_db_xchg_words (P.mb_w, P.mb_h) + (expand ? border_lds : 0), P.db_num_bands);
+    return expand;
   }
   void run_scene (const WhSeqParams& P, const WhPicJob* jobs, int n) override {
     hipLaunchKernelGGL (k_scene, dim3 (P.mb_w * P.mb_h, n), dim3 (64), 0, stream_, P, jobs);
diff --git a/openh264_amd/csrc/host/backend.h b/openh264_amd/csrc/host/backend.h
--- a/openh264_amd/csrc/host/backend.h
+++ b/openh264_amd/csrc/host/backend.h
@@ -28,6 +28,7 @@
   virtual void run_scene (const WhSeqParams& P, const WhPicJob* jobs, int n) = 0;
   virtual void run_qp_chain (const WhSeqParams& P, const WhPicJob* jobs, int n) = 0;
   virtual void run_deblock (const WhSeqParams& P, const WhPicJob* jobs, int n) = 0;
+  virtual bool run_deblock_expand (const WhSeqParams& P, const WhPicJob* jobs, int n) { run_deblock (P, jobs, n); return false; }
   virtual void run_expand (const WhSeqParams& P, const WhPicJob* jobs, int n) = 0;
   virtual void run_compact (const WhSeqParams& P, const WhPicJob* jobs, int n) = 0;
   virtual void run_sse (const WhSeqParams& P, const WhPicJob* jobs, int n);
@@ -50,6 +51,13 @@
   virtual float event_elapsed_ms (void* a, void* b) = 0;
 };
 
+inline bool run_deblock_and_expand (Backend* be, const WhSeqParams& P, const WhPicJob* jobs, int n, bool deblock, bool expand) {
+  bool fused = false;
+  if (deblock) { if (expand) fused = be->run_deblock_expand (P, jobs, n); else be->run_deblock (P, jobs, n); }
+  if (expand && !fused) be->run_expand (P, jobs, n);
+  return fused;
+}
+
 Backend* create_hip_backend (int device, const char** err);
 
 }
diff --git a/openh264_amd/csrc/host/encoder.cpp b/openh264_amd/csrc/host/encoder.cpp
--- a/openh264_amd/csrc/host/encoder.cpp
+++ b/openh264_amd/csrc/host/encoder.cpp
@@ -644,8 +644,7 @@
   if (idr) be->run_intra (s, d_jobs, n);
   else be->run_inter (s, d_jobs, n);
   if (qp_map && s.deblock_idc != 1) be->run_qp_chain (s, d_jobs, n);
-  if (s.deblock_idc != 1) be->run_deblock (s, d_jobs, n);
-  if (need_ref) be->run_expand (s, d_jobs, n);
+  wh::run_deblock_and_expand (be, s, d_jobs, n, s.deblock_idc != 1, need_ref);
   if (sse) be->run_sse (s, d_jobs, n);
 }
 
@@ -1063,8 +1062,7 @@
     if (np) g->be->run_inter (plain_seq (s), g->d_jobs + a, np);
     if (ni) g->be->run_intra (s, g->d_jobs + a + np, ni);
     if (c0.use_compact) g->be->run_compact (s, g->d_jobs + a, b - a);
-    if (s.deblock_idc != 1) g->be->run_deblock (s, g->d_jobs + a, b - a);
-    if (c0.prm.uiIntraPeriod != 1) g->be->run_expand (s, g->d_jobs + a, b - a);
+    wh::run_deblock_and_expand (g->be, s, g->d_jobs + a, b - a, s.deblock_idc != 1, c0.prm.uiIntraPeriod != 1);
     if (g->sse_planes()) g->be->run_sse (s, g->d_jobs + a, b - a);
   }
   if (wait && g->be->sync()) { set_err ("device scheduler timed out"); return WELSHIP_ERR_UNKNOWN; }
@@ -1246,8 +1244,7 @@
   if (np) be->run_inter (plain_seq (s), dj, np);
   if (n - np) be->run_intra (s, dj + np, n - np);
   be->run_compact (s, dj, n);
-  if (s.deblock_idc != 1) be->run_deblock (s, dj, n);
-  if (c0.prm.uiIntraPeriod != 1) be->run_expand (s, dj, n);
+  wh::run_deblock_and_expand (be, s, dj, n, s.deblock_idc != 1, c0.prm.uiIntraPeriod != 1);
   if (sse) be->run_sse (s, dj, n);
   be->event_record (g->step_ev[sb]);
   for (auto& c : g->sess) c->submit_advance();
@@ -1298,8 +1295,7 @@
   be->upload (g->d_job_aux, job, sizeof (WhPicJob));
   if (idr) be->run_intra (c.seq, g->d_job_aux, 1); else be->run_inter (c.seq, g->d_job_aux, 1);
   be->run_compact (c.seq, g->d_job_aux, 1);
-  if (c.seq.deblock_idc != 1) be->run_deblock (c.seq, g->d_job_aux, 1);
-  if (c.prm.uiIntraPeriod != 1) be->run_expand (c.seq, g->d_job_aux, 1);
+  wh::run_deblock_and_expand (be, c.seq, g->d_job_aux, 1, c.seq.deblock_idc != 1, c.prm.uiIntraPeriod != 1);
   if (job->sse_planes) { be->fill (job->sse, 0, 3 * sizeof (uint64_t)); be->run_sse (c.seq, g->d_job_aux, 1); }
   if (be->sync()) { set_err ("device scheduler timed out; the picture was not encoded"); return WELSHIP_ERR_UNKNOWN; }
   return WELSHIP_OK;
@@ -1423,9 +1419,10 @@
       if (q == 0) be->event_record (ev[i * 4 + 0]);
       if (g->step_idr) be->run_intra (s, g->d_jobs + a, cnt); else be->run_inter (plain_seq (s), g->d_jobs + a, cnt);
       if (q == 0) be->event_record (ev[i * 4 + 1]);
-      if (s.deblock_idc != 1) be->run_deblock (s, g->d_jobs + a, cnt);
+      bool fused = false;
+      if (s.deblock_idc != 1) { if (need_ref) fused = be->run_deblock_expand (s, g->d_jobs + a, cnt); else be->run_deblock (s, g->d_jobs + a, cnt); }
       if (q == 0) be->event_record (ev[i * 4 + 2]);
-      if (need_ref) be->run_expand (s, g->d_jobs + a, cnt);
+      if (need_ref && !fused) be->run_expand (s, g->d_jobs + a, cnt);
       if (q == 0) be->event_record (ev[i * 4 + 3]);
       if (g->sse_planes()) be->run_sse (s, g->d_jobs + a, cnt);
     }
diff --git a/openh264_amd/csrc/host/frame_api.cpp b/openh264_amd/csrc/host/frame_api.cpp
--- a/openh264_amd/csrc/host/frame_api.cpp
+++ b/openh264_amd/csrc/host/frame_api.cpp
@@ -326,8 +326,7 @@
       be->err_snapshot (q, L->h_err.data());
       be->event_record_on (q, L->tail_ev);
     }
-    if (s.deblock_idc != 1) be->run_deblock (s, L->d_jobs, n);
-    if (K->expand) be->run_expand (s, L->d_jobs, n);
+    wh::run_deblock_and_expand (be, s, L->d_jobs, n, s.deblock_idc != 1, K->expand);
     for (FrameItem* x : batch) x->c->tail_queue = tail && L->tail_ev ? q : -1;
     if (tail && L->tail_ev) {
       if (L->h_err_tail.empty()) { L->h_err_tail.assign (8, 0u); be->pin_host (L->h_err_tail.data(), 32); for (void*& e : L->tail_done_ev) e = be->event_create(); }
@@ -840,8 +839,7 @@
     if (last_part) {
       job.mb_begin = 0; job.mb_end = 0; be->sync_queue (queue); be->upload (c->d_job, &job, sizeof (job));
       if (qp_map) be->run_qp_chain (s, c->d_job, 1);
-      if (s.deblock_idc != 1) be->run_deblock (s, c->d_job, 1);
-      if (j->bExpand) be->run_expand (s, c->d_job, 1);
+      wh::run_deblock_and_expand (be, s, c->d_job, 1, s.deblock_idc != 1, j->bExpand != 0);
       cur.is_p = is_p;
       if (dyn) std::swap (c->d_sad_cost0, c->d_sad_cost0_new);
       if (j->pSadCost) be->download (j->pSadCost, c->d_sad_cost0, sizeof (int32_t) * c->num_mb);
diff --git a/openh264_amd/csrc/kernels/border_pic.h b/openh264_amd/csrc/kernels/border_pic.h
--- /dev/null
+++ b/openh264_amd/csrc/kernels/border_pic.h
@@ -0,0 +1,139 @@
+#pragma once
+#include "expand_pic.h"
+#include "tile_pic.h"
+
+#define WH_BORDER_GROUP 4
+#define WH_BORDER_MAX_DEPS 5
+#define WH_BORDER_BATCH 4
+
+typedef struct WhBorderChunk {
+  int kind;
+  int bottom, right;
+  int k0, k1;
+  int deps[WH_BORDER_MAX_DEPS];
+} WhBorderChunk;
+
+WH_HDFN int wh_border_groups (const WhSeqParams& P) { return (P.mb_w + WH_BORDER_GROUP - 1) / WH_BORDER_GROUP; }
+WH_HDFN int wh_border_chunks (const WhSeqParams& P) { return 2 * wh_border_groups (P) + 4 + P.mb_h; }
+
+WH_HDFN WhBorderChunk wh_border_chunk (const WhSeqParams& P, int id) {
+  const int w = P.mb_w, h = P.mb_h, ng = wh_border_groups (P);
+  WhBorderChunk C;
+  C.kind = 0; C.bottom = 0; C.right = 0; C.k0 = 0; C.k1 = 0;
+  C.deps[0] = C.deps[1] = C.deps[2] = C.deps[3] = C.deps[4] = -1;
+  if (id >= ng + 2 && id < ng + 2 + h) {
+    const int y = id - (ng + 2), below = y + 1 < h;
+    C.kind = 2; C.k0 = y;
+    C.deps[0] = y * w;
+    C.deps[1] = w > 1 ? y * w + w - 1 : -1;
+    C.deps[2] = below ? (y + 1) * w : -1;
+    C.deps[3] = below && w > 1 ? (y + 1) * w + w - 1 : -1;
+    return C;
+  }
+  if (id >= ng + 2 + h) { C.bottom = 1; id -= ng + 2 + h; }
+  const int row = C.bottom ? (h - 1) * w : 0;
+  if (id < ng) {
+    C.k0 = id * WH_BORDER_GROUP; C.k1 = C.k0 + WH_BORDER_GROUP < w ? C.k0 + WH_BORDER_GROUP : w;
+    C.deps[0] = row + C.k0;
+    C.deps[1] = C.k0 + 1 <= C.k1 && C.k0 + 1 < w ? row + C.k0 + 1 : -1;
+    C.deps[2] = C.k0 + 2 <= C.k1 && C.k0 + 2 < w ? row + C.k0 + 2 : -1;
+    C.deps[3] = C.k0 + 3 <= C.k1 && C.k0 + 3 < w ? row + C.k0 + 3 : -1;
+    C.deps[4] = C.k0 + 4 <= C.k1 && C.k0 + 4 < w ? row + C.k0 + 4 : -1;
+    return C;
+  }
+  C.kind = 1; C.right = id - ng;
+  C.deps[0] = row + (C.right ? w - 1 : 0);
+  return C;
+}
+
+WH_HDFN void wh_border_tb_range (const WhBorderChunk& C, int mbs, int w, int pad, int* x0, int* x1) {
+  if (C.kind == 0) { *x0 = C.k0 * mbs; *x1 = C.k1 * mbs; }
+  else { *x0 = C.right ? w : -pad; *x1 = *x0 + pad; }
+}
+WH_HDFN int wh_border_expand_items_pl (const WhSeqParams& P, const WhBorderChunk& C, int pl) {
+  int w, h, pad, stride;
+  wh_expand_plane_geom (P, pl, &w, &h, &pad, &stride);
+  const int mbs = pl == 0 ? 16 : 8;
+  if (C.kind == 2) return mbs * (pad >> 1);
+  int x0, x1;
+  wh_border_tb_range (C, mbs, w, pad, &x0, &x1);
+  return pad * ((x1 - x0) >> 2);
+}
+WH_HDFN int wh_border_expand_items (const WhSeqParams& P, const WhBorderChunk& C) {
+  return wh_border_expand_items_pl (P, C, 0) + 2 * wh_border_expand_items_pl (P, C, 1);
+}
+WH_HDFN uint32_t wh_border_expand_op (const WhSeqParams& P, const WhPicJob& J, const WhBorderChunk& C, int i, bool store, uint32_t v) {
+  int pl = 0;
+  const int n0 = wh_border_expand_items_pl (P, C, 0);
+  if (i >= n0) { const int n1 = wh_border_expand_items_pl (P, C, 1); i -= n0; pl = 1; if (i >= n1) { i -= n1; pl = 2; } }
+  int w, h, pad, stride;
+  wh_expand_plane_geom (P, pl, &w, &h, &pad, &stride);
+  WH_G uint8_t* base = (WH_G uint8_t*)J.rec[pl];
+  const int mbs = pl == 0 ? 16 : 8;
+  if (C.kind == 2) {
+    const int per_row = pad >> 1, per_side = pad >> 2;
+    const int rr = i / per_row, k = i - rr * per_row, right = k >= per_side, j = k - right * per_side, r = C.k0 * mbs + rr;
+    if (!store) return wh_expand_side_value (base, stride, w, r, right);
+    wh_expand_side_store (base, stride, w, pad, r, right, j, v);
+    return 0;
+  }
+  int x0, x1;
+  wh_border_tb_range (C, mbs, w, pad, &x0, &x1);
+  const int per_row = (x1 - x0) >> 2;
+  const int rr = i / per_row, x = x0 + 4 * (i - rr * per_row), r = (C.bottom ? pad : 0) + rr;
+  if (!store) return wh_expand_tb_value (base, stride, w, h, pad, r, x);
+  wh_expand_tb_store (base, stride, h, pad, r, x, v);
+  return 0;
+}
+
+WH_HDFN void wh_border_tile_rect (const WhSeqParams& P, const WhBorderChunk& C, int pl, int* tx0, int* tx1, int* ty0, int* ty1) {
+  const int tw = pl == 0 ? P.rec_stride_y >> 4 : P.rec_stride_c >> 3;
+  const int top = pl == 0 ? 4 : 2, per_mb = pl == 0 ? 2 : 1, th = top + per_mb * P.mb_h + top;
+  if (C.kind == 2) { *tx0 = 0; *tx1 = tw; *ty0 = top + per_mb * C.k0; *ty1 = *ty0 + per_mb; return; }
+  *ty0 = C.bottom ? th - top : 0; *ty1 = *ty0 + top;
+  if (C.kind == 0) { *tx0 = 2 + C.k0; *tx1 = 2 + C.k1; }
+  else if (!C.right) { *tx0 = 0; *tx1 = 2; }
+  else { *tx0 = 2 + P.mb_w; *tx1 = tw; }
+}
+WH_HDFN int wh_border_tile_items_pl (const WhSeqParams& P, const WhBorderChunk& C, int pl) {
+  int tx0, tx1, ty0, ty1;
+  wh_border_tile_rect (P, C, pl, &tx0, &tx1, &ty0, &ty1);
+  return 8 * (ty1 - ty0) * (C.kind == 2 ? tx1 - tx0 - P.mb_w : tx1 - tx0);
+}
+WH_HDFN int wh_border_tile_items (const WhSeqParams& P, const WhBorderChunk& C) { return wh_border_tile_items_pl (P, C, 0) + wh_border_tile_items_pl (P, C, 1); }
+WH_HDFN WhU4 wh_border_tile_op (const WhSeqParams& P, const WhPicJob& J, const WhBorderChunk& C, int i, bool store, WhU4 v) {
+  int pl = 0;
+  const int n0 = wh_border_tile_items_pl (P, C, 0);
+  if (i >= n0) { i -= n0; pl = 1; }
+  int tx0, tx1, ty0, ty1;
+  wh_border_tile_rect (P, C, pl, &tx0, &tx1, &ty0, &ty1);
+  const int cols = C.kind == 2 ? tx1 - tx0 - P.mb_w : tx1 - tx0;
+  const int row = i & 7, t = i >> 3, tr = t / cols, tc = t - tr * cols;
+  const int ty = ty0 + tr, tx = C.kind == 2 ? (tc < 2 ? tc : tc + P.mb_w) : tx0 + tc;
+  if (!store) return pl == 0 ? wh_tile_row_y (P, J, tx, ty, row) : wh_tile_row_c (P, J, tx, ty, row);
+  if (pl == 0) wh_tile_put_y (P, J, tx, ty, row, v); else wh_tile_put_c (P, J, tx, ty, row, v);
+  return v;
+}
+
+WH_HDFN void wh_border_chunk_expand (const WhSeqParams& P, const WhPicJob& J, const WhBorderChunk& C, int lane, int lanes) {
+  const int n = wh_border_expand_items (P, C);
+  for (int i0 = lane; i0 < n; i0 += lanes * WH_BORDER_BATCH) {
+    uint32_t v[WH_BORDER_BATCH];
+#pragma unroll
+    for (int u = 0; u < WH_BORDER_BATCH; ++u) if (i0 + u * lanes < n) v[u] = wh_border_expand_op (P, J, C, i0 + u * lanes, false, 0u);
+#pragma unroll
+    for (int u = 0; u < WH_BORDER_BATCH; ++u) if (i0 + u * lanes < n) (void)wh_border_expand_op (P, J, C, i0 + u * lanes, true, v[u]);
+  }
+}
+WH_HDFN void wh_border_chunk_tiles (const WhSeqParams& P, const WhPicJob& J, const WhBorderChunk& C, int lane, int lanes) {
+  const int n = wh_border_tile_items (P, C);
+  for (int i0 = lane; i0 < n; i0 += lanes * WH_BORDER_BATCH) {
+    WhU4 v[WH_BORDER_BATCH];
+    WhU4 none;
+    none.x = none.y = none.z = none.w = 0u;
+#pragma unroll
+    for (int u = 0; u < WH_BORDER_BATCH; ++u) if (i0 + u * lanes < n) v[u] = wh_border_tile_op (P, J, C, i0 + u * lanes, false, none);
+#pragma unroll
+    for (int u = 0; u < WH_BORDER_BATCH; ++u) if (i0 + u * lanes < n) (void)wh_border_tile_op (P, J, C, i0 + u * lanes, true, v[u]);
+  }
+}
diff --git a/openh264_amd/csrc/kernels/expand_pic.h b/openh264_amd/csrc/kernels/expand_pic.h
--- a/openh264_amd/csrc/kernels/expand_pic.h
+++ b/openh264_amd/csrc/kernels/expand_pic.h
@@ -8,6 +8,20 @@
 WH_HDFN int wh_expand_plane_items (int w, int h, int pad) { return h * (pad >> 1) + 2 * pad * ((w + 2 * pad) >> 2); }
 WH_HDFN int wh_expand_items (const WhSeqParams& P) {
   return wh_expand_plane_items (P.mb_w * 16, P.mb_h * 16, 32) + 2 * wh_expand_plane_items (P.mb_w * 8, P.mb_h * 8, 16);
+}
+
+WH_HDFN uint32_t wh_expand_side_value (const WH_G uint8_t* base, int stride, int w, int r, int right) {
+  return 0x01010101u * base[(ptrdiff_t)r * stride + (right ? w - 1 : 0)];
+}
+WH_HDFN void wh_expand_side_store (WH_G uint8_t* base, int stride, int w, int pad, int r, int right, int j, uint32_t v) {
+  * (WH_G uint32_t*) (base + (ptrdiff_t)r * stride + (right ? w + 4 * j : -pad + 4 * j)) = v;
+}
+WH_HDFN uint32_t wh_expand_tb_value (const WH_G uint8_t* base, int stride, int w, int h, int pad, int r, int x) {
+  const WH_G uint8_t* srow = base + (ptrdiff_t) (r < pad ? 0 : h - 1) * stride;
+  return x < 0 ? 0x01010101u * srow[0] : x >= w ? 0x01010101u * srow[w - 1] : * (const WH_G uint32_t*) (srow + x);
+}
+WH_HDFN void wh_expand_tb_store (WH_G uint8_t* base, int stride, int h, int pad, int r, int x, uint32_t v) {
+  * (WH_G uint32_t*) (base + (ptrdiff_t) (r < pad ? r - pad : h + r - pad) * stride + x) = v;
 }
 
 WH_HDFN void wh_expand_item (const WhSeqParams& P, WH_G uint8_t* rec0, WH_G uint8_t* rec1, WH_G uint8_t* rec2, int idx) {
@@ -25,15 +39,11 @@
   const int side_items = h * (pad >> 1), per_side = pad >> 2;
   if (idx < side_items) {
     const int r = idx / (2 * per_side), k = idx - r * 2 * per_side, right = k >= per_side, j = k - right * per_side;
-    const uint32_t v = 0x01010101u * base[(ptrdiff_t)r * stride + (right ? w - 1 : 0)];
-    * (WH_G uint32_t*) (base + (ptrdiff_t)r * stride + (right ? w + 4 * j : -pad + 4 * j)) = v;
+    wh_expand_side_store (base, stride, w, pad, r, right, j, wh_expand_side_value (base, stride, w, r, right));
     return;
   }
   idx -= side_items;
   const int per_row = (w + 2 * pad) >> 2;
   const int r = idx / per_row, x = -pad + 4 * (idx - r * per_row);
-  const bool top = r < pad;
-  const WH_G uint8_t* srow = base + (ptrdiff_t) (top ? 0 : h - 1) * stride;
-  const uint32_t v = x < 0 ? 0x01010101u * srow[0] : x >= w ? 0x01010101u * srow[w - 1] : * (const WH_G uint32_t*) (srow + x);
-  * (WH_G uint32_t*) (base + (ptrdiff_t) (top ? r - pad : h + r - pad) * stride + x) = v;
+  wh_expand_tb_store (base, stride, h, pad, r, x, wh_expand_tb_value (base, stride, w, h, pad, r, x));
 }
diff --git a/openh264_amd/csrc/kernels/tile_pic.h b/openh264_amd/csrc/kernels/tile_pic.h
--- a/openh264_amd/csrc/kernels/tile_pic.h
+++ b/openh264_amd/csrc/kernels/tile_pic.h
@@ -5,20 +5,25 @@
 WH_HDFN int wh_tile_items_c (const WhSeqParams& P) { return (P.rec_stride_c >> 3) * ((P.mb_h * 8 + 32) >> 3) * 8; }
 WH_HDFN int wh_tile_items (const WhSeqParams& P) { return wh_tile_items_y (P) + wh_tile_items_c (P); }
 
-WH_HDFN void wh_tile_copy_y (const WhSeqParams& P, const WhPicJob& J, int tx, int ty, int row) {
-  const int tw = P.rec_stride_y >> 4;
-  const WH_G uint8_t* src = (const WH_G uint8_t*)J.rec[0] - (ptrdiff_t)32 * P.rec_stride_y - 32 + (ptrdiff_t) (ty * 8 + row) * P.rec_stride_y + tx * 16;
-  wh_stg16 ((WH_G uint8_t*)J.rec_tiles[0] + ((size_t) (ty * tw + tx) * 8 + row) * 16, wh_ldg16 (src));
+WH_HDFN WhU4 wh_tile_row_y (const WhSeqParams& P, const WhPicJob& J, int tx, int ty, int row) {
+  return wh_ldg16 ((const WH_G uint8_t*)J.rec[0] - (ptrdiff_t)32 * P.rec_stride_y - 32 + (ptrdiff_t) (ty * 8 + row) * P.rec_stride_y + tx * 16);
 }
-WH_HDFN void wh_tile_copy_c (const WhSeqParams& P, const WhPicJob& J, int tx, int ty, int row) {
-  const int tw = P.rec_stride_c >> 3;
+WH_HDFN void wh_tile_put_y (const WhSeqParams& P, const WhPicJob& J, int tx, int ty, int row, WhU4 v) {
+  wh_stg16 ((WH_G uint8_t*)J.rec_tiles[0] + ((size_t) (ty * (P.rec_stride_y >> 4) + tx) * 8 + row) * 16, v);
+}
+WH_HDFN WhU4 wh_tile_row_c (const WhSeqParams& P, const WhPicJob& J, int tx, int ty, int row) {
   const ptrdiff_t off = - (ptrdiff_t)16 * P.rec_stride_c - 16 + (ptrdiff_t) (ty * 8 + row) * P.rec_stride_c + tx * 8;
   const WH_G uint32_t* cb = (const WH_G uint32_t*) ((const WH_G uint8_t*)J.rec[1] + off);
   const WH_G uint32_t* cr = (const WH_G uint32_t*) ((const WH_G uint8_t*)J.rec[2] + off);
   WhU4 v;
   v.x = cb[0]; v.y = cb[1]; v.z = cr[0]; v.w = cr[1];
-  wh_stg16 ((WH_G uint8_t*)J.rec_tiles[1] + ((size_t) (ty * tw + tx) * 8 + row) * 16, v);
+  return v;
 }
+WH_HDFN void wh_tile_put_c (const WhSeqParams& P, const WhPicJob& J, int tx, int ty, int row, WhU4 v) {
+  wh_stg16 ((WH_G uint8_t*)J.rec_tiles[1] + ((size_t) (ty * (P.rec_stride_c >> 3) + tx) * 8 + row) * 16, v);
+}
+WH_HDFN void wh_tile_copy_y (const WhSeqParams& P, const WhPicJob& J, int tx, int ty, int row) { wh_tile_put_y (P, J, tx, ty, row, wh_tile_row_y (P, J, tx, ty, row)); }
+WH_HDFN void wh_tile_copy_c (const WhSeqParams& P, const WhPicJob& J, int tx, int ty, int row) { wh_tile_put_c (P, J, tx, ty, row, wh_tile_row_c (P, J, tx, ty, row)); }
 WH_HDFN void wh_tile_item (const WhSeqParams& P, const WhPicJob& J, int idx) {
   const int ny = wh_tile_items_y (P);
   if (idx < ny) { const int tw = P.rec_stride_y >> 4, tile = idx >> 3; wh_tile_copy_y (P, J, tile % tw, tile / tw, idx & 7); return; }
```

Result: no change. 27900 (median of 6 runs) (+0.4%).
